# rti-team-imvia/RNb-NeuS-fork

Hardware: AMD Instinct MI355X
Metric: training rays/sec at 512 rays x 128 samples/ray (higher is better)
Workload: dtype f32; 1 GPU; DiLiGenT-MV-shaped synthetic rays, wmask_rnb.conf networks (8x256 SDF MLP + 2x256 albedo MLP), train_rnb step (render_rnb), 512 rays x (64+64) samples per GPU, 3 lights, geometric init, Adam; rays_per_gpu=512, global_rays=512, samples_per_ray=128, n_lights=3, no_albedo=False, parallelism=dp1, dp_loss=single process, deterministic=False, arithmetic=x2h, operand_bits=22, train_ops=rnb_loss_rnb + rnb_adam_step (one launch each)

## Files before the change

include/rnbneus.h:

```cpp
#ifndef RNBNEUS_H
#define RNBNEUS_H

#include <stddef.h>
#include <stdint.h>

#ifdef __cplusplus
extern "C" {
#endif

#define RNB_ABI_VERSION 5
#define RNB_MAX_LIN 16

enum {
  RNB_OK = 0,
  RNB_E_INVALID = -1,
  RNB_E_WORKSPACE = -2,
  RNB_E_HIP = -3,
  RNB_E_NULL = -4
};

typedef void* rnb_stream_t;

typedef struct rnb_model_desc {
  int32_t sdf_d_in;
  int32_t sdf_d_out;
  int32_t sdf_d_hidden;
  int32_t sdf_n_layers;
  int32_t sdf_skip_in;
  int32_t sdf_multires;
  float   sdf_scale;
  int32_t sdf_weight_norm;
  int32_t col_d_feature;
  int32_t col_d_in;
  int32_t col_d_out;
  int32_t col_d_hidden;
  int32_t col_n_layers;
  int32_t col_multires_view;
  int32_t col_squeeze_out;
  int32_t col_weight_norm;
  int32_t n_samples;
  int32_t n_importance;
  int32_t up_sample_steps;
  int32_t variant;
} rnb_model_desc;

enum {
  RNB_VARIANT_BF16 = 1,
  RNB_VARIANT_DETERMINISTIC = 2,
  RNB_VARIANT_GENERIC = 4,
  RNB_VARIANT_DW_LDS = 8,
  RNB_VARIANT_DW_STAGED = 16,
  RNB_VARIANT_X3 = 32,
  RNB_VARIANT_F32_MFMA = 64,
  RNB_VARIANT_BWD_TI_SHIFT = 8,
  RNB_VARIANT_BWD_NW_SHIFT = 10,
  RNB_VARIANT_FWD_TI_SHIFT = 12,
  RNB_VARIANT_FWD_NW_SHIFT = 14,
  RNB_VARIANT_REG_TILE = 1 << 16,
  RNB_VARIANT_LDS_TILE = 1 << 17,
  RNB_VARIANT_X2H = 1 << 18,
  RNB_VARIANT_NO_X2H = 1 << 19
};

typedef struct rnb_mlp_params {
  int32_t n_lin;
  int32_t pad_;
  const float* g[RNB_MAX_LIN];
  const float* v[RNB_MAX_LIN];
  const float* b[RNB_MAX_LIN];
} rnb_mlp_params;

typedef struct rnb_mlp_grads {
  int32_t n_lin;
  int32_t pad_;
  float* g[RNB_MAX_LIN];
  float* v[RNB_MAX_LIN];
  float* b[RNB_MAX_LIN];
} rnb_mlp_grads;

int rnb_abi_version(void);
const char* rnb_build_id(void);
const char* rnb_last_error_string(void);

int rnb_packed_floats(const rnb_model_desc* desc, int64_t* n_floats);
int rnb_weightnorm_fwd(const rnb_model_desc* desc, const rnb_mlp_params* sdf, const rnb_mlp_params* color,
                       float* packed, rnb_stream_t stream);
int rnb_weightnorm_bwd(const rnb_model_desc* desc, const rnb_mlp_params* sdf, const rnb_mlp_params* color,
                       const float* packed_grad, const rnb_mlp_grads* sdf_grads,
                       const rnb_mlp_grads* color_grads, rnb_stream_t stream);

int rnb_points_workspace_bytes(const rnb_model_desc* desc, int64_t n_points, int64_t* bytes);
int rnb_sdf_forward(const rnb_model_desc* desc, const float* packed, const float* pts, int64_t n,
                    float* sdf_out, float* feat_out, void* ws, size_t ws_bytes, rnb_stream_t stream);
int rnb_sdf_gradient(const rnb_model_desc* desc, const float* packed, const float* pts, int64_t n,
                     float* grad_out, float* sdf_out, void* ws, size_t ws_bytes, rnb_stream_t stream);
int rnb_color_forward(const rnb_model_desc* desc, const float* packed, const float* pts,
                      const float* normals, const float* feats, int64_t n, float* out, void* ws,
                      size_t ws_bytes, rnb_stream_t stream);

enum { RNB_POINTS_FEATURE = 1, RNB_POINTS_NORMAL = 2, RNB_POINTS_COLOR = 4 };
int rnb_points_grad_workspace_bytes(const rnb_model_desc* desc, int64_t n_points, int32_t flags, int64_t* bytes);
int rnb_sdf_forward_save(const rnb_model_desc* desc, const float* packed, const float* pts, int64_t n,
                         int32_t flags, float* sdf_out, float* feat_out, float* nrm_out, void* ws, size_t ws_bytes,
                         rnb_stream_t stream);
int rnb_sdf_backward(const rnb_model_desc* desc, const float* packed, int64_t n, int32_t flags, const float* sdf_bar,
                     const float* feat_bar, const float* nrm_bar, float* packed_grad, float* x_bar, void* ws,
                     size_t ws_bytes, rnb_stream_t stream);
int rnb_color_forward_save(const rnb_model_desc* desc, const float* packed, const float* pts, const float* normals,
                           const float* feats, int64_t n, float* out, void* ws, size_t ws_bytes, rnb_stream_t stream);
int rnb_color_backward(const rnb_model_desc* desc, const float* packed, int64_t n, const float* alb_bar,
                       float* packed_grad, float* feat_bar, float* nrm_bar, float* pts_bar, void* ws, size_t ws_bytes,
                       rnb_stream_t stream);

typedef struct rnb_grid_desc {
  float bound_min[3];
  float bound_max[3];
  int32_t resolution;
  int32_t x_begin, x_end;
  float out_scale;
} rnb_grid_desc;
int rnb_sdf_grid_workspace_bytes(const rnb_model_desc* desc, const rnb_grid_desc* grid, int64_t* bytes);
int rnb_sdf_grid(const rnb_model_desc* desc, const float* packed, const rnb_grid_desc* grid, float* volume,
                 void* ws, size_t ws_bytes, rnb_stream_t stream);

typedef struct rnb_sparse_grid_desc {
  int32_t brick;
  float threshold;
  float margin;
} rnb_sparse_grid_desc;
int rnb_sdf_grid_sparse_workspace_bytes(const rnb_model_desc* desc, const rnb_grid_desc* grid,
                                        const rnb_sparse_grid_desc* sparse, int64_t* bytes);
int rnb_sdf_grid_sparse_seed(const rnb_model_desc* desc, const float* packed, const rnb_grid_desc* grid,
                             const rnb_sparse_grid_desc* sparse, void* ws, size_t ws_bytes, int64_t* n_listed,
                             rnb_stream_t stream);
int rnb_sdf_grid_sparse_round(const rnb_model_desc* desc, const float* packed, const rnb_grid_desc* grid,
                              const rnb_sparse_grid_desc* sparse, float* volume, void* ws, size_t ws_bytes, int64_t first,
                              int64_t count, int64_t* n_listed, rnb_stream_t stream);
int rnb_sdf_grid_sparse_finish(const rnb_model_desc* desc, const rnb_grid_desc* grid, const rnb_sparse_grid_desc* sparse,
                               float* volume, void* ws, size_t ws_bytes, uint8_t* brick_mask, rnb_stream_t stream);

int rnb_up_sample_step(const float* rays_o, const float* rays_d, const float* z_in, const float* sdf_in,
                       int64_t B, int32_t n, int32_t n_new, float inv_s, float* new_z, int32_t* inds,
                       float* z_out, int32_t* sort_index, rnb_stream_t stream);
int rnb_gather_sdf(const float* sdf_old, const float* sdf_new, const int32_t* sort_index, int64_t B,
                   int32_t n, int32_t n_new, float* sdf_out, rnb_stream_t stream);
int rnb_sample_workspace_bytes(const rnb_model_desc* desc, int64_t B, int64_t* bytes);
int rnb_sample_rays(const rnb_model_desc* desc, const float* packed, const float* rays_o,
                    const float* rays_d, const float* near, const float* far, const float* t_rand,
                    int64_t B, float* z_vals_out, void* ws, size_t ws_bytes, rnb_stream_t stream);

enum {
  RNB_MODE_CORE = 0,
  RNB_MODE_MVPS = 1,
  RNB_FLAG_RELU_SHADING = 2,
  RNB_FLAG_NO_ALBEDO = 4,
  RNB_FLAG_LIGHT_PER_RAY = 8,
  RNB_FLAG_FORWARD_ONLY = 16,
  RNB_FLAG_INPUT_GRADS = 32
};

typedef struct rnb_render_args {
  int64_t B;
  int32_t S;
  int32_t n_lights;
  int32_t flags;
  float   cos_anneal_ratio;
  const float* rays_o;
  const float* rays_d;
  const float* z_vals;
  const float* lights_dir;
  const float* background_rgb;
  const float* variance;
  float* color_fine;
  float* weights;
  float* cdf_fine;
  float* gradients;
  float* inside_sphere;
  float* weight_sum;
  float* weight_max;
  float* s_val;
  float* gradient_error;
  float* sdf;
  float* sampled_albedo;
  float* gerr_partial;
  const float* gerr_den_global;
} rnb_render_args;

typedef struct rnb_render_grads {
  const float* color_fine;
  const float* weights;
  const float* cdf_fine;
  const float* gradients;
  const float* weight_sum;
  const float* weight_max;
  const float* s_val;
  const float* gradient_error;
} rnb_render_grads;

int rnb_render_workspace_bytes(const rnb_model_desc* desc, int64_t B, int32_t S, int32_t flags,
                               int64_t* bytes);
int rnb_render_fwd(const rnb_model_desc* desc, const float* packed, const rnb_render_args* args,
                   void* ws, size_t ws_bytes, rnb_stream_t stream);
int rnb_render_bwd(const rnb_model_desc* desc, const float* packed, const rnb_render_args* args,
                   const rnb_render_grads* gout, float* packed_grad, float* variance_grad, void* ws,
                   size_t ws_bytes, rnb_stream_t stream);

typedef struct rnb_render_input_grads {
  float* rays_o;
  float* rays_d;
  float* lights_dir;
  float* background_rgb;
  float* z_vals;
} rnb_render_input_grads;

int rnb_render_bwd_inputs(const rnb_model_desc* desc, const float* packed, const rnb_render_args* args,
                          const rnb_render_grads* gout, const rnb_render_input_grads* igrads, float* packed_grad,
                          float* variance_grad, void* ws, size_t ws_bytes, rnb_stream_t stream);

typedef struct rnb_render_maps_out {
  float* color;
  float* normal;
  float* albedo;
  float* depth;
  float* weight_sum;
  float* weight_max;
} rnb_render_maps_out;
int rnb_render_maps(const rnb_model_desc* desc, const float* packed, const rnb_render_args* args,
                    const rnb_render_maps_out* maps, void* ws, size_t ws_bytes, rnb_stream_t stream);

int rnb_algorithmic_flops(const rnb_model_desc* desc, int64_t B, int32_t flags, double* train_flops,
                          double* forward_flops);

int rnb_algorithmic_bytes(const rnb_model_desc* desc, int64_t B, int32_t flags, double* train_bytes);

int rnb_marching_cubes_workspace_bytes(int32_t nx, int32_t ny, int32_t nz, int64_t* bytes);
int rnb_marching_cubes_count(const float* volume, int32_t nx, int32_t ny, int32_t nz, float threshold,
                             void* workspace, size_t workspace_bytes, int64_t* counts, rnb_stream_t stream);
int rnb_marching_cubes_emit(const float* volume, int32_t nx, int32_t ny, int32_t nz, float threshold,
                            void* workspace, size_t workspace_bytes, int64_t n_vertices, int64_t n_triangles,
                            double* vertices, int32_t* triangles, rnb_stream_t stream);

enum { RNB_MESH_ALBEDO = 1, RNB_MESH_SWAP_RB = 2 };
typedef struct rnb_mesh_vertex_args {
  const double* grid_vertices;
  const float* points;
  int64_t V;
  float bound_min[3], bound_max[3];
  int32_t resolution;
  float level;
  int32_t refine;
  float max_step;
  int32_t flags;
  float* points_out;
  float* sdf_out;
  float* gradient_out;
  float* normal_out;
  float* albedo_out;
  uint8_t* rgb_out;
} rnb_mesh_vertex_args;
int rnb_mesh_vertex_workspace_bytes(const rnb_model_desc* desc, int64_t chunk, int32_t flags, int64_t* bytes);
int rnb_mesh_vertex_attrs(const rnb_model_desc* desc, const float* packed, const rnb_mesh_vertex_args* args,
                          int64_t chunk, void* ws, size_t ws_bytes, rnb_stream_t stream);

int rnb_gen_rays_at_view(const float* intrinsics_inv, const float* pose, const float* images,
                         const float* images_warmup, const float* mask, int32_t mask_channels,
                         const float* light_directions, const int64_t* pixels_x, const int64_t* pixels_y, int64_t B,
                         int32_t n_lights, int32_t H, int32_t W, float* data, float* true_rgb,
                         float* true_rgb_warmup, float* lights_dir, float* near, float* far, rnb_stream_t stream);

int rnb_gen_rays_grid(const float* intrinsics_inv, const float* pose, const float* tx, const float* ty, int32_t Wl,
                      int32_t Hl, int64_t first, int64_t n, const float* images, const float* images_warmup,
                      const float* mask, int32_t mask_channels, const float* light_directions, int32_t n_lights,
                      int32_t light, int32_t H, int32_t W, float* data, float* true_rgb, float* true_rgb_warmup,
                      float* lights_dir, float* near, float* far, rnb_stream_t stream);

enum { RNB_SOURCE_U8 = 0, RNB_SOURCE_U16 = 1, RNB_SOURCE_F32 = 2 };
typedef struct rnb_source_maps {
  const void* normals;
  const void* albedo;
  const void* mask;
  int32_t normals_type;
  int32_t mask_type;
  int32_t H, W, mask_channels;
  int32_t n_lights;
  float local_lights[8][3];
  float warmup_lights_cam[8][3];
} rnb_source_maps_t;
int rnb_gen_rays_at_view_from_maps(const float* intrinsics_inv, const float* pose, const rnb_source_maps_t* source,
                                   const int64_t* pixels_x, const int64_t* pixels_y, int64_t B, float* data,
                                   float* true_rgb, float* true_rgb_warmup, float* lights_dir, float* near, float* far,
                                   rnb_stream_t stream);
int rnb_gen_rays_grid_from_maps(const float* intrinsics_inv, const float* pose, const float* view_pose, const float* tx,
                                const float* ty, int32_t Wl, int32_t Hl, int64_t first, int64_t n,
                                const rnb_source_maps_t* source, int32_t light, float* data, float* true_rgb,
                                float* true_rgb_warmup, float* lights_dir, float* near, float* far, rnb_stream_t stream);

int rnb_gen_rays_camera_bwd(const float* intrinsics_inv, const float* pose, const int64_t* pixels_x,
                            const int64_t* pixels_y, int64_t B, const float* lights_dir, int32_t n_lights,
                            const float* rays_o_bar, const float* rays_d_bar, const float* lights_bar,
                            const float* near_bar, const float* far_bar, float* pose_bar, float* intrinsics_inv_bar,
                            rnb_stream_t stream);

int rnb_loss_rnb(const float* color_fine, const float* true_rgb, const float* mask, const float* weight_sum,
                 const float* gradient_error, int32_t n_lights, int64_t B, int32_t color_depth, float igr_weight,
                 float mask_weight, float* loss, float* parts, float* d_color_fine, float* d_weight_sum,
                 float* d_gradient_error, rnb_stream_t stream);
int rnb_loss_rnb_shard(const float* color_fine, const float* true_rgb, const float* mask, const float* weight_sum,
                       const float* gradient_error, int32_t n_lights, int64_t B, int32_t color_depth, float igr_weight,
                       float mask_weight, const float* batch_global, float eik_share,
                       float* loss, float* parts, float* d_color_fine, float* d_weight_sum, float* d_gradient_error,
                       rnb_stream_t stream);

int rnb_adam_step(float* param, const float* grad, float* exp_avg, float* exp_avg_sq, int64_t n, double lr,
                  double beta1, double beta2, double eps, double weight_decay, int64_t step, rnb_stream_t stream);

int rnb_render_range(const rnb_model_desc* desc, const float* packed, const void* ws, size_t ws_bytes, int64_t B, int32_t S,
                     int32_t flags, float* out, rnb_stream_t stream);

int rnb_profile_enable(int on);
int rnb_profile_collect(double* gemm_ms, int64_t* gemm_launches, double* gemm_flops);
int64_t rnb_profile_report(char* out, int64_t capacity);

#ifdef __cplusplus
}
#endif
#endif
```

rnb-neus-fork_amd/csrc/backward.hip:

```cpp
#include "gemm.hip.h"
#include "pe.hip.h"
#include "rnb_internal.h"

namespace rnb {

__global__ __launch_bounds__(64) void nbar_geb_kernel(const float* __restrict__ x4, const float* __restrict__ nrm,
                                                      const float* __restrict__ nbar_in,
                                                      const float* __restrict__ cinb, int Cinp, int blk_off,
                                                      int pen_off, int multires_view, int with_color, int multires,
                                                      int Ep, int64_t M, int64_t Mp, float* __restrict__ geb,
                                                      unsigned* __restrict__ amax) {
  extern __shared__ float tile[];
  const int lane = threadIdx.x;
  const int64_t r0 = (int64_t)blockIdx.x * 64, row = r0 + lane;
  float nb[3] = {0.f, 0.f, 0.f};
  if (with_color) {
    const int Wc = Cinp - blk_off;
    tile_load64(cinb, Cinp, r0, blk_off, Wc, tile, lane);
    __builtin_amdgcn_wave_barrier();
    if (row < M) {
      const float* g = tile + lane * (Wc + 1) + (pen_off - blk_off);
#pragma unroll
      for (int d = 0; d < 3; ++d) nb[d] = nbar_in[row * 4 + d] + g[d];
      pe_adjoint(nrm + row * 4, g, multires_view, 0, 1, nb);
    }
    __builtin_amdgcn_wave_barrier();
  } else if (row < M) {
#pragma unroll
    for (int d = 0; d < 3; ++d) nb[d] = nbar_in[row * 4 + d];
  }
  float* o = tile + lane * (Ep + 1);
  o[0] = nb[0]; o[1] = nb[1]; o[2] = nb[2];
  float gm = fmaxf(fmaxf(fabsf(nb[0]), fabsf(nb[1])), fabsf(nb[2]));
  pe_tangent(x4 + row * 4, nb, multires, 0, 1, [&](int c, float v0, float v1) {
    o[c] = v0;
    o[c + 3] = v1;
    gm = fmaxf(gm, fmaxf(fabsf(v0), fabsf(v1)));
  });
  for (int c = 3 + 6 * multires; c < Ep; ++c) o[c] = 0.f;
  if (amax != nullptr) amax_commit(amax, gm, lane);
  __builtin_amdgcn_wave_barrier();
  tile_store64(geb, Ep, r0, 0, Ep, tile, lane);
}

__global__ __launch_bounds__(512) void sdf_head_bwd_kernel(const float* __restrict__ a, const float* __restrict__ ulast,
                                                           const float* __restrict__ ucol, int ntiles,
                                                           int Hp, int H, const float* __restrict__ sbar,
                                                           float inv_scale, int64_t M, int rows_per_blk,
                                                           float* __restrict__ dwsdf, float* __restrict__ dbsdf,
                                                           float* __restrict__ part_w, float* __restrict__ part_b) {
  __shared__ double red[64][33];
  __shared__ double redb[64];
  const int tid = threadIdx.x, cg = tid & 7, ph = tid >> 3;
  const int kl = cg * 4, k0 = blockIdx.y * 32 + kl;
  const int64_t r0 = (int64_t)blockIdx.x * rows_per_blk;
  const int64_t r1 = min(M, r0 + rows_per_blk);
  double s[4] = {0.0, 0.0, 0.0, 0.0}, sb = 0.0;
#pragma unroll 4
  for (int64_t row = r0 + ph; row < r1; row += 64) {
    const float t = sbar[row] * inv_scale;
    if (cg == 0) sb += (double)t;
    const vf4 av = *reinterpret_cast<const vf4*>(a + row * Hp + k0);
    if (ulast != nullptr) {
      const vf4 uv = *reinterpret_cast<const vf4*>(ulast + row * Hp + k0);
#pragma unroll
      for (int j = 0; j < 4; ++j) s[j] += (double)(t * av[j] + uv[j]);
    } else {
#pragma unroll
      for (int j = 0; j < 4; ++j) s[j] += (double)(t * av[j]);
    }
  }
  if (ulast == nullptr && blockIdx.x == 0) {
    for (int tile = ph; tile < ntiles; tile += 64) {
      const vf4 uv = *reinterpret_cast<const vf4*>(ucol + (size_t)tile * Hp + k0);
#pragma unroll
      for (int j = 0; j < 4; ++j) s[j] += (double)uv[j];
    }
  }
#pragma unroll
  for (int j = 0; j < 4; ++j) red[ph][kl + j] = s[j];
  if (cg == 0) redb[ph] = sb;
  __syncthreads();
  if (tid < 32) {
    double t = 0.0;
    for (int q = 0; q < 64; ++q) t += red[q][tid];
    const int col = blockIdx.y * 32 + tid;
    if (part_w != nullptr) part_w[(size_t)blockIdx.x * Hp + col] = col < H ? (float)t : 0.f;
    else if (col < H) atomicAdd(dwsdf + col, (float)t);
  } else if (tid == 32 && blockIdx.y == 0) {
    double t = 0.0;
    for (int q = 0; q < 64; ++q) t += redb[q];
    if (part_b != nullptr) part_b[blockIdx.x] = (float)t;
    else atomicAdd(dbsdf, (float)t);
  }
}

__global__ void sdf_xbar_kernel(const float* __restrict__ x4, const float* __restrict__ ebar, const float* __restrict__ ge,
                                const float* __restrict__ nbar, int Ep, int multires, float scale, int64_t M,
                                float* __restrict__ xbar) {
  const int64_t row = (int64_t)blockIdx.x * blockDim.x + threadIdx.x;
  if (row >= M) return;
  const float* eb = ebar + row * Ep;
  float acc[3] = {eb[0], eb[1], eb[2]};
  const float* g = ge != nullptr ? ge + row * Ep : nullptr;
  pe_adjoint_hess(x4 + row * 4, eb, g != nullptr, g, nbar + row * 4, multires, 0, 1, acc);
#pragma unroll
  for (int d = 0; d < 3; ++d) xbar[row * 3 + d] = scale * acc[d];
}

__global__ void color_input_bwd_kernel(const float* __restrict__ cinb, int Cinp, int F, int pev, int multires_view,
                                       const float* __restrict__ p4, const float* __restrict__ n4, int64_t M,
                                       float* __restrict__ pbar, float* __restrict__ nbar) {
  const int64_t row = (int64_t)blockIdx.x * blockDim.x + threadIdx.x;
  if (row >= M) return;
  for (int which = 0; which < 2; ++which) {
    float* out = which ? nbar : pbar;
    if (out == nullptr) continue;
    const float* g = cinb + row * Cinp + F + which * pev;
    const float* v = (which ? n4 : p4) + row * 4;
    float t[3] = {g[0], g[1], g[2]};
    pe_adjoint(v, g, multires_view, 0, 1, t);
#pragma unroll
    for (int d = 0; d < 3; ++d) out[row * 3 + d] = t[d];
  }
}


static int launch_nbar_geb(const Layout& L, PointBufs& pb, bool with_color, hipStream_t s) {
  const int wt = (with_color && L.Cinp - L.F > L.Ep) ? L.Cinp - L.F : L.Ep;
  hipLaunchKernelGGL(nbar_geb_kernel, dim3(blocks_for(pb.Mp, 64)), dim3(64), (size_t)64 * (wt + 1) * sizeof(float), s,
                     pb.x, pb.nrm, pb.nbar, pb.cinb, L.Cinp, L.F, L.F + L.pev, L.multires_view, with_color ? 1 : 0,
                     L.multires, L.Ep, pb.M, pb.Mp, pb.geb, (unsigned*)nullptr);
  RNB_CHECK_LAUNCH();
  return RNB_OK;
}

static int launch_sdf_head_bwd(const Layout& L, PointBufs& pb, bool u_rows, int u_tiles, float* packed_grad, int* slabs_out,
                               hipStream_t s) {
  const int64_t M = pb.M;
  const int chunks = L.Hp / 32;
  int64_t slabs = (L.variant & RNB_VARIANT_DETERMINISTIC) ? 1 : (256 + chunks - 1) / chunks;
  const bool slab_out = dw_one_wg_runs(L, M);
  if (slab_out) slabs = kSdfHeadSlabs;
  int rows_per_blk = (int)((M + slabs - 1) / slabs);
  rows_per_blk = (rows_per_blk + 63) / 64 * 64;
  const unsigned nslab = blocks_for(M, rows_per_blk);
  hipLaunchKernelGGL(sdf_head_bwd_kernel, dim3(nslab, chunks), dim3(512), 0, s, pb.a[L.nh - 1],
                     u_rows ? (const float*)pb.u[L.nh] : (const float*)nullptr, (const float*)pb.u[L.nh], u_tiles, L.Hp,
                     L.H, pb.sbar, 1.f / L.sdf_scale, M, rows_per_blk, packed_grad + L.wsdf_off, packed_grad + L.bsdf_off,
                     slab_out ? pb.sdfh_part : nullptr, slab_out ? pb.sdfh_part + (size_t)nslab * L.Hp : nullptr);
  RNB_CHECK_LAUNCH();
  *slabs_out = slab_out ? (int)nslab : 0;
  return RNB_OK;
}

static int check_route_buffers(const Layout& L, const PointBufs& pb, const BwdParts& parts) {
  const Route& r = L.route;
  const char* missing = nullptr;
  if (r.h2 && pb.amax == nullptr) missing = "amax";
  else if (r.h2 && pb.smax == nullptr) missing = "smax";
  else if (parts.albedo && r.color == COLOR_BF16 && pb.cin8 == nullptr) missing = "cin8";
  else if (parts.albedo && r.color == COLOR_H2 && pb.col_part == nullptr) missing = "col_part";
  else if (parts.sdf && r.sdf != SDF_BF16 && dw_one_wg_runs(L, pb.M) && pb.sdfh_part == nullptr) missing = "sdfh_part";
  if (missing != nullptr) RNB_FAIL(RNB_E_WORKSPACE, "backward: this workspace has no PointBufs::%s, which the model's kernel route needs", missing);
  return RNB_OK;
}


int sweep_backward(const Layout& L, const float* packed, PointBufs& pb, bool with_color, float* packed_grad, hipStream_t s) {
  return sweep_backward_parts(L, packed, pb, BwdParts::render(with_color, false), packed_grad, s);
}

int sweep_backward_parts(const Layout& L, const float* packed, PointBufs& pb, const BwdParts& parts, float* packed_grad,
                         hipStream_t s) {
  const Route& r = L.route;
  RNB_TRY(check_route_buffers(L, pb, parts));
  RNB_TRY(dw_zero_partials(L, pb, s));
  BwdParts dw_parts = parts;
  dw_parts.albedo = parts.albedo && r.color != COLOR_BF16;
  if (parts.albedo) switch (r.color) {
    case COLOR_BF16: RNB_TRY(bf16_color_backward(L, packed, pb, packed_grad, s)); break;
    case COLOR_H2: RNB_TRY(color_h2_backward(L, packed, pb, s, parts.sdf, parts.color_inputs)); break;
    case COLOR_LAYERS: RNB_TRY(layers_color_backward(L, packed, pb, packed_grad, s)); break;
    case COLOR_NONE: RNB_FAIL(RNB_E_INVALID, "backward: the model has no albedo network");
  }
  if (!parts.sdf) return dw_backward(L, pb, dw_parts, 0, packed_grad, s);
  if (parts.normal && !(parts.albedo && r.color == COLOR_H2)) RNB_TRY(launch_nbar_geb(L, pb, parts.albedo, s));
  const bool bf = r.sdf == SDF_BF16;
  if (bf) {
    dw_parts.sdf = false;
    RNB_TRY(dw_backward(L, pb, dw_parts, 0, packed_grad, s));
  }
  int u_tiles = 0;
  if (bf) {
    RNB_TRY(bf16_ra(L, packed, pb, s));
  } else if (!parts.normal) {
    for (int l = 0; l < L.nh; ++l) RNB_CHECK_HIP(hipMemsetAsync(pb.zR[l], 0, (size_t)pb.Mp * L.Hp * sizeof(float), s));
  } else if (r.sdf == SDF_FUSED) {
    RNB_TRY(fused_ra(L, packed, pb, s, &u_tiles));
  } else {
    RNB_TRY(layers_ra(L, packed, pb, s));
  }
  int sdfh_slabs = 0;
  if (bf) RNB_TRY(bf16_sdf_head_bwd(L, pb, packed_grad, s));
  else RNB_TRY(launch_sdf_head_bwd(L, pb, parts.normal && r.sdf == SDF_LAYERS, u_tiles, packed_grad, &sdfh_slabs, s));
  switch (r.sdf) {
    case SDF_BF16: RNB_TRY(bf16_fb(L, packed, pb, parts.albedo, s)); break;
    case SDF_FUSED: RNB_TRY(fused_fb(L, packed, pb, parts.feat, s)); break;
    case SDF_LAYERS: RNB_TRY(layers_fb(L, packed, pb, parts.feat, s)); break;
  }
  if (bf) return bf16_dw_backward(L, pb, parts.albedo, packed_grad, s);
  return dw_backward(L, pb, dw_parts, sdfh_slabs, packed_grad, s);
}


int launch_sdf_xbar(const Layout& L, const float* packed, PointBufs& pb, bool with_normal, float* xbar, hipStream_t s) {
  float* ebar = nullptr;
  RNB_TRY(launch_sdf_ebar(L, packed, pb, &ebar, s));
  hipLaunchKernelGGL(sdf_xbar_kernel, dim3(blocks_for(pb.M, 256)), dim3(256), 0, s, pb.x, ebar,
                     with_normal ? (const float*)pb.ge : nullptr, pb.nbar, L.Ep, L.multires, L.sdf_scale, pb.M, xbar);
  RNB_CHECK_LAUNCH();
  return RNB_OK;
}

int launch_color_input_bwd(const Layout& L, const PointBufs& pb, float* pts_bar, float* nrm_bar, hipStream_t s) {
  if (pts_bar == nullptr && nrm_bar == nullptr) return RNB_OK;
  hipLaunchKernelGGL(color_input_bwd_kernel, dim3(blocks_for(pb.M, 256)), dim3(256), 0, s, pb.cinb, L.Cinp, L.F, L.pev,
                     L.multires_view, pb.x, pb.nrm, pb.M, pts_bar, nrm_bar);
  RNB_CHECK_LAUNCH();
  return RNB_OK;
}

}
```

rnb-neus-fork_amd/csrc/fused_bwd.hip:

```cpp
#include "fused_common.hip.h"
#include "pe.hip.h"

namespace rnb {


struct FusedBwdArgs {
  const float* packed;
  const x3raw* w3;
  SdfNetArgs net;
  float* D[RNB_MAX_LIN];
  float* gz[RNB_MAX_LIN];
  float* u[RNB_MAX_LIN + 1];
  long long M;
  float* ucol;
  float* zR[RNB_MAX_LIN];
  float* zb[RNB_MAX_LIN];
  const float* x4;
  float* nrm;
  const float* geb;
  const float* sbar;
  const float* fbar;
  int ld_fbar;
  unsigned* amax;
  const H2Tab* h2tab;
  unsigned* smax;
  float* ge_out;
};

template <int TI, int TJ = 2, bool X3 = false, class Hook = NoHook, int NP = 3>
__device__ inline void layer_mma(const float* __restrict__ X, const FusedBwdArgs& g, long long off, int K, int n0, int lane,
                                 v16f (&acc)[TI][TJ], X3Mma<TI, TJ, NP>& mm, long long off_next, Hook hook = Hook(),
                                 int hook_late = 0) {
  if constexpr (X3 && TI == 2 && TJ == 2) {
    mm.request(g.w3 + NP * off, K, n0, lane);
    mm.run(X, g.w3 + NP * off, K, n0, lane, acc, nullptr, 0, 0, hook);
  } else if constexpr (X3) mm.run(X, g.w3 + NP * off, K, n0, lane, acc, off_next >= 0 ? g.w3 + NP * off_next : nullptr, FH, n0, hook);
  else if constexpr (TI == 2 && TJ == 2) layer_mma_nt_ring<TI>(X, g.packed + off, K, n0, lane, acc, hook);
  else layer_mma_nt<TI, Hook, TJ>(X, g.packed + off, K, n0, lane, acc, hook, hook_late);
}

template <int TI, int NW = 4, bool X3 = false, bool H2 = false>
__global__ __launch_bounds__(64 * NW, (NW == 8 && TI == 2) ? 1 : 2) void fused_reverse_kernel(FusedBwdArgs g) {
  static_assert(!H2 || X3, "x2h is a form of the split-operand path");
  constexpr float SG = H2 ? kH2ActScale : 1.f;
  constexpr int WP = H2 ? 2 : 3;
  constexpr int BT = 32 * TI;
  constexpr int NT = 64 * NW;
  constexpr int TJ = 8 / NW;
  [[maybe_unused]] constexpr bool BOTH_IN_LOOP = !(TI == 2 && TJ == 2);
  constexpr int NBUF = TI == 1 ? 2 : 1;
  __shared__ __attribute__((aligned(16))) float lds[NBUF * BT * FP + BT * FEP];
  __shared__ float wmx[8];
  __shared__ int ovf[2];
  float* X = lds;
  float* Y = lds + (NBUF - 1) * BT * FP;
  float* GE = lds + NBUF * BT * FP;
  const int tid = threadIdx.x, lane = tid & 63;
  const int wave = wave_id();
  const int64_t row0 = (int64_t)blockIdx.x * BT;
  const int n0 = wave * 32 * TJ;
  [[maybe_unused]] float sg = SG, isg = 1.f / SG;
  [[maybe_unused]] float iwsv = 0.f;
  if constexpr (H2) iwsv = h2_iws_load(g.h2tab, lane);

  [[maybe_unused]] float sm = 0.f;
  {
    const float* Dl = g.D[g.net.nh - 1] + (size_t)row0 * FH;
    float* gzl = g.gz[g.net.nh - 1] + (size_t)row0 * FH;
    const float* ws = g.packed + g.net.wsdf_off;
    float m = 0.f;
    for (int idx = tid; idx < BT * FH / 4; idx += NT) {
      const int r = idx >> 6, c4 = idx & 63;
      const vf4 d = *reinterpret_cast<const vf4*>(Dl + r * FH + c4 * 4);
      const vf4 w = *reinterpret_cast<const vf4*>(ws + c4 * 4);
      const vf4 v = d * w;
      *reinterpret_cast<vf4*>(X + r * FP + c4 * 4) = v * SG;
      *reinterpret_cast<vf4*>(gzl + r * FH + c4 * 4) = v;
      if constexpr (H2) m = fmaxf(fmaxf(m, fmaxf(fabsf(v.x), fabsf(v.y))), fmaxf(fabsf(v.z), fabsf(v.w)));
    }
    for (int idx = tid; idx < BT * FEP; idx += NT) GE[idx] = 0.f;
    if constexpr (H2) {
      const bool any = __builtin_amdgcn_ballot_w64(m >= kH2ActLimit) != 0;
      if (lane == 0) wmx[wave] = any ? 1.f : 0.f;
      if (tid < 2) ovf[tid] = 0;
    }
    if constexpr (H2) sm = m;
  }
  __syncthreads();
  if constexpr (H2) {
    if (tile_max<NW>(wmx) != 0.f) {
      __syncthreads();
      sm = wave_max(sm);
      if (lane == 0) wmx[wave] = sm;
      __syncthreads();
      const float tm = tile_max<NW>(wmx);
      if (g.smax != nullptr && tid == 0) amax_tile_commit(g.smax + SMAX_GZ + g.net.nh - 1, tm);
      x2h_dyn_scale(__builtin_bit_cast(unsigned, tm), sg, isg);
      const float f = sg * (1.f / SG);
      for (int idx = tid; idx < BT * FH / 4; idx += NT) {
        vf4* q = reinterpret_cast<vf4*>(X + (idx >> 6) * FP + (idx & 63) * 4);
        *q = *q * f;
      }
      __syncthreads();
    }
  }

  v16f acc[TI][TJ];
  AuxTile<TI, TJ> aD;
  [[maybe_unused]] X3Mma<TI, TJ, WP> mm;
  if constexpr (X3 && !(TI == 2 && TJ == 2)) {
    if (g.net.nh > 1 || n0 < 64) mm.request(g.w3 + WP * g.net.wT_off[g.net.nh - 1], FH, n0, lane);
  }
  for (int l = g.net.nh - 1; l >= 1; --l) {
    [[maybe_unused]] const float INV = H2 ? isg * h2_iws_at(iwsv, l) : 1.f;
    const long long nxt = (l > 1 || n0 < 64) ? g.net.wT_off[l - 1] : -1;
    constexpr bool LATE = X3 && TI == 2 && TJ == 2;
    layer_mma<TI, TJ, X3>(X, g, g.net.wT_off[l], FH, n0, lane, acc, mm, nxt,
                     [&]() { if constexpr (!LATE) prefetch_tile<TI, TJ>(g.D[l - 1], row0, n0, lane, aD); });
    const int lane_e = opaque_lane(lane);
    const int h = lane_e >> 5;
    if constexpr (LATE) prefetch_tile<TI, TJ>(g.D[l - 1], row0, n0, lane_e, aD);
    if constexpr (NBUF == 1) lds_barrier();
    const bool is_skip = (l == g.net.skip);
    const int ksplit = is_skip ? FH - g.net.pe : FH;
    const BufRsrc rg = tile_rsrc(g.gz[l - 1] + (size_t)row0 * FH, BT * FH * 4);
    [[maybe_unused]] float gm[2] = {0.f, 0.f};
    for_each_acc_split<TI, TJ>(
        n0, lane_e, ksplit,
        [&](int tj, int ti, int r, int col, int rowc, int row) {
          const float gzv = acc[ti][tj][r] * INV * aD.v[ti][tj][r];
          Y[row * FP + col] = gzv * SG;
          bstore(rg, (unsigned)(4 * h * FH + col) * 4u, rowc * FH * 4, gzv);
          if constexpr (H2) gm[r & 1] = fmaxf(gm[r & 1], fabsf(gzv));
        },
        [&](int tj, int ti, int r, int col, int rowc, int row) {
          const float v = acc[ti][tj][r] * INV;
          float gzv;
          if (col < ksplit) {
            gzv = v * aD.v[ti][tj][r];
          } else {
            if (col < ksplit + g.net.pe) GE[row * FEP + (col - ksplit)] = v;
            gzv = 0.f;
          }
          Y[row * FP + col] = gzv * SG;
          bstore(rg, (unsigned)(4 * h * FH + col) * 4u, rowc * FH * 4, gzv);
          if constexpr (H2) gm[r & 1] = fmaxf(gm[r & 1], fabsf(gzv));
        });
    if constexpr (H2) h2_raise_flag(fmaxf(gm[0], gm[1]), &ovf[l & 1], lane_e);
    lds_barrier();
    if constexpr (H2) {
      sg = SG;
      isg = 1.f / SG;
      if (h2_flag_up(&ovf[l & 1])) {
        const float m = wave_max(fmaxf(gm[0], gm[1]));
        if (lane_e == 0) wmx[wave] = m;
        lds_barrier();
        const float tm = tile_max<NW>(wmx);
        if (g.smax != nullptr && tid == 0) amax_tile_commit(g.smax + SMAX_GZ + l - 1, tm);
        if (tid == 0) ovf[l & 1] = 0;
        x2h_dyn_scale(__builtin_bit_cast(unsigned, tm), sg, isg);
        const float f = sg * (1.f / SG);
        for_each_acc<TI, TJ>(n0, lane_e, [&](int tj, int ti, int r, int col, int rowc, int row) { Y[row * FP + col] *= f; });
        lds_barrier();
      }
    }
    if constexpr (NBUF == 2) { float* t = X; X = Y; Y = t; }
  }
  if (n0 < 64) {
    [[maybe_unused]] const float INV = H2 ? isg * h2_iws_at(iwsv, 0) : 1.f;
    layer_mma<TI, TJ, X3>(X, g, g.net.wT_off[0], FH, n0, lane, acc, mm, -1);
    for_each_acc<TI, TJ>(n0, lane, [&](int tj, int ti, int r, int col, int rowc, int row) {
      if (col < g.net.pe) GE[row * FEP + col] += acc[ti][tj][r] * INV;
    });
  }
  __syncthreads();
  if (tid < BT) {
    const int64_t row = row0 + tid;
    const float* ge = GE + tid * FEP;
    float n[3] = {ge[0], ge[1], ge[2]};
    pe_adjoint(g.x4 + row * 4, ge, g.net.multires, 0, 1, n);
    g.nrm[row * 4] = n[0]; g.nrm[row * 4 + 1] = n[1]; g.nrm[row * 4 + 2] = n[2]; g.nrm[row * 4 + 3] = 0.f;
    if (g.ge_out != nullptr)
      for (int c = 0; c < g.net.pe; ++c) g.ge_out[row * g.net.Ep + c] = ge[c];
  }
}

template <int TI, int NW = 4, bool X3 = false>
__global__ __launch_bounds__(64 * NW, (NW == 8 && TI == 2) ? 1 : 2) void fused_ra_kernel(FusedBwdArgs g) {
  constexpr int BT = 32 * TI;
  constexpr int NT = 64 * NW;
  constexpr int TJ = 8 / NW;
  [[maybe_unused]] constexpr bool BOTH_IN_LOOP = !(TI == 2 && TJ == 2);
  constexpr int NBUF = TI == 1 ? 2 : 1;
  __shared__ __attribute__((aligned(16))) float lds[NBUF * BT * FP + BT * FEP];
  float* X = lds;
  float* Y = lds + (NBUF - 1) * BT * FP;
  float* E = lds + NBUF * BT * FP;
  __shared__ float wmx[2][8];
  const int tid = threadIdx.x, lane = tid & 63;
  const int wave = wave_id();
  const int64_t row0 = (int64_t)blockIdx.x * BT;
  const int n0 = wave * 32 * TJ;

  float gm = 0.f;
  for (int idx = tid; idx < BT * g.net.Ep; idx += NT) {
    const int r = idx / g.net.Ep, c = idx - r * g.net.Ep;
    const float v = g.geb[(row0 + r) * g.net.Ep + c];
    X[r * FP + c] = v;
    if (c < FEP) E[r * FEP + c] = v;
    gm = fmaxf(gm, fabsf(v));
  }
  if (g.amax != nullptr) {
#pragma unroll
    for (int o = 32; o > 0; o >>= 1) gm = fmaxf(gm, __shfl_xor(gm, o, 64));
    if (lane == 0) wmx[1][wave] = gm;
  }
  __syncthreads();
  if (g.amax != nullptr && tid == 0) {
    float m = wmx[1][0];
    for (int w = 1; w < NW; ++w) m = fmaxf(m, wmx[1][w]);
    amax_tile_commit(g.amax + AMAX_U, m);
  }

  v16f acc[TI][TJ];
  AuxTile<TI, TJ> aD, aG;
  [[maybe_unused]] X3Mma<TI, TJ> mm;
  if constexpr (X3 && !(TI == 2 && TJ == 2)) mm.request(g.w3 + 3 * g.net.w_off[0], g.net.Kp[0], n0, lane);
  for (int l = 0; l < g.net.nh; ++l) {
    layer_mma<TI, TJ, X3>(X, g, g.net.w_off[l], g.net.Kp[l], n0, lane, acc, mm, l + 1 < g.net.nh ? g.net.w_off[l + 1] : -1,
                     [&]() {
                       if constexpr (!(X3 && !BOTH_IN_LOOP)) prefetch_tile<TI, TJ>(g.D[l], row0, n0, lane, aD);
                       if constexpr (BOTH_IN_LOOP) prefetch_tile<TI, TJ>(g.gz[l], row0, n0, lane, aG);
                     });
    const int lane_e = opaque_lane(lane);
    const int h = lane_e >> 5;
    if constexpr (X3 && !BOTH_IN_LOOP) prefetch_tile<TI, TJ>(g.D[l], row0, n0, lane_e, aD);
    if constexpr (!BOTH_IN_LOOP) prefetch_tile<TI, TJ>(g.gz[l], row0, n0, lane_e, aG);
    if constexpr (NBUF == 1) lds_barrier();
    const int n_real = g.net.n_real[l];
    const bool pe_tail = (l + 1 == g.net.skip);
    const BufRsrc rzR = tile_rsrc(g.zR[l] + (size_t)row0 * FH, BT * FH * 4);
    if (l + 1 == g.net.nh && g.ucol != nullptr) {
      float cs[TJ];
#pragma unroll
      for (int tj = 0; tj < TJ; ++tj) cs[tj] = 0.f;
      for_each_acc<TI, TJ>(n0, lane_e, [&](int tj, int ti, int r, int col, int rowc, int row) {
        const float v = acc[ti][tj][r];
        const float un = col < n_real ? v * aD.v[ti][tj][r] : 0.f;
        const float zr = col < n_real ? ((v - un) * aG.v[ti][tj][r]) * 100.f : 0.f;
        bstore(rzR, (unsigned)(4 * h * FH + col) * 4u, rowc * FH * 4, zr);
        cs[tj] += (row0 + row < g.M) ? un : 0.f;
      });
#pragma unroll
      for (int tj = 0; tj < TJ; ++tj) {
        const float tot = cs[tj] + __shfl_xor(cs[tj], 32, 64);
        if (lane_e < 32) g.ucol[(size_t)blockIdx.x * FH + n0 + tj * 32 + lane_e] = tot;
      }
      break;
    }
    const BufRsrc ru = tile_rsrc(g.u[l + 1] + (size_t)row0 * FH, BT * FH * 4);
    float um[2] = {0.f, 0.f};
    for_each_acc_split<TI, TJ>(
        n0, lane_e, n_real,
        [&](int tj, int ti, int r, int col, int rowc, int row) {
          const unsigned voff = (unsigned)(4 * h * FH + col) * 4u;
          const unsigned soff = rowc * FH * 4;
          const float v = acc[ti][tj][r];
          const float un = v * aD.v[ti][tj][r];
          const float zr = ((v - un) * aG.v[ti][tj][r]) * 100.f;
          Y[row * FP + col] = un;
          bstore(rzR, voff, soff, zr);
          bstore(ru, voff, soff, un);
          um[r & 1] = fmaxf(um[r & 1], fabsf(un));
        },
        [&](int tj, int ti, int r, int col, int rowc, int row) {
          const unsigned voff = (unsigned)(4 * h * FH + col) * 4u;
          const unsigned soff = rowc * FH * 4;
          const float v = acc[ti][tj][r];
          float zr, un;
          if (col < n_real) {
            un = v * aD.v[ti][tj][r];
            zr = ((v - un) * aG.v[ti][tj][r]) * 100.f;
          } else {
            zr = 0.f;
            un = (pe_tail && col < n_real + g.net.pe) ? E[row * FEP + (col - n_real)] : 0.f;
          }
          Y[row * FP + col] = un;
          bstore(rzR, voff, soff, zr);
          bstore(ru, voff, soff, un);
          um[r & 1] = fmaxf(um[r & 1], fabsf(un));
        });
    if (g.amax != nullptr) {
      float m = fmaxf(um[0], um[1]);
#pragma unroll
      for (int o = 32; o > 0; o >>= 1) m = fmaxf(m, __shfl_xor(m, o, 64));
      if (lane_e == 0) wmx[l & 1][wave] = m;
    }
    lds_barrier();
    if (g.amax != nullptr && tid == 0) {
      float m = wmx[l & 1][0];
      for (int w = 1; w < NW; ++w) m = fmaxf(m, wmx[l & 1][w]);
      amax_tile_commit(g.amax + AMAX_U + l + 1, m);
    }
    if constexpr (NBUF == 2) { float* t = X; X = Y; Y = t; }
  }
}

template <int TI, int NW = 4, bool X3 = false>
__global__ __launch_bounds__(64 * NW, (NW == 8 && TI == 2) ? 1 : 2) void fused_fb_kernel(FusedBwdArgs g) {
  constexpr int BT = 32 * TI;
  constexpr int NT = 64 * NW;
  constexpr int TJ = 8 / NW;
  [[maybe_unused]] constexpr bool BOTH_IN_LOOP = !(TI == 2 && TJ == 2);
  constexpr int NBUF = TI == 1 ? 2 : 1;
  __shared__ __attribute__((aligned(16))) float lds[NBUF * BT * FP];
  float* X = lds;
  float* Y = lds + (NBUF - 1) * BT * FP;
  const int tid = threadIdx.x, lane = tid & 63;
  const int wave = wave_id();
  const int64_t row0 = (int64_t)blockIdx.x * BT;
  const int n0 = wave * 32 * TJ;

  v16f acc[TI][TJ];
  AuxTile<TI, TJ> aD, aZ;
  [[maybe_unused]] X3Mma<TI, TJ> mm;
  if constexpr (X3 && !(TI == 2 && TJ == 2)) {
    if (g.fbar != nullptr) mm.request(g.w3 + 3 * g.net.wfT_off, FH, n0, lane);
    else if (g.net.nh > 1) mm.request(g.w3 + 3 * g.net.wT_off[g.net.nh - 1], FH, n0, lane);
  }
  constexpr bool LATE = X3 && TI == 2 && TJ == 2;
  if constexpr (!LATE) {
    prefetch_tile<TI, TJ>(g.D[g.net.nh - 1], row0, n0, lane, aD);
    prefetch_tile<TI, TJ>(g.zR[g.net.nh - 1], row0, n0, lane, aZ);
  }
  for (int ti_ = 0; ti_ < TI; ++ti_) for (int tj_ = 0; tj_ < TJ; ++tj_) for (int r_ = 0; r_ < 16; ++r_) acc[ti_][tj_][r_] = 0.f;
  if (g.fbar != nullptr) {
    const float* fb = g.fbar + (size_t)row0 * g.ld_fbar;
    for (int idx = tid; idx < BT * FH / 4; idx += NT) {
      const int r = idx >> 6, c4 = idx & 63;
      *reinterpret_cast<vf4*>(X + r * FP + c4 * 4) = *reinterpret_cast<const vf4*>(fb + (size_t)r * g.ld_fbar + c4 * 4);
    }
    __syncthreads();
    layer_mma<TI, TJ, X3>(X, g, g.net.wfT_off, FH, n0, lane, acc, mm, g.net.nh > 1 ? g.net.wT_off[g.net.nh - 1] : -1);
    if constexpr (NBUF == 1) lds_barrier();
  }
  if constexpr (LATE) {
    prefetch_tile<TI, TJ>(g.D[g.net.nh - 1], row0, n0, lane, aD);
    prefetch_tile<TI, TJ>(g.zR[g.net.nh - 1], row0, n0, lane, aZ);
  }
  for (int l = g.net.nh - 1; l >= 0; --l) {
    const int lane_e = opaque_lane(lane);
    const int h = lane_e >> 5;
    const int n_real = g.net.n_real[l];
    const bool head = (l == g.net.nh - 1);
    const BufRsrc rzb = tile_rsrc(g.zb[l] + (size_t)row0 * FH, BT * FH * 4);
    if (head) {
      for_each_acc<TI, TJ>(n0, lane_e, [&](int tj, int ti, int r, int col, int rowc, int row) {
        acc[ti][tj][r] = fmaf(g.sbar[row0 + row] * g.net.inv_scale, g.packed[g.net.wsdf_off + col], acc[ti][tj][r]);
      });
    }
    for_each_acc_split<TI, TJ>(
        n0, lane_e, n_real,
        [&](int tj, int ti, int r, int col, int rowc, int row) {
          const float zb = fmaf(acc[ti][tj][r], aD.v[ti][tj][r], aZ.v[ti][tj][r]);
          Y[row * FP + col] = zb;
          bstore(rzb, (unsigned)(4 * h * FH + col) * 4u, rowc * FH * 4, zb);
          acc[ti][tj][r] = zb;
        },
        [&](int tj, int ti, int r, int col, int rowc, int row) {
          const float zb = col < n_real ? fmaf(acc[ti][tj][r], aD.v[ti][tj][r], aZ.v[ti][tj][r]) : 0.f;
          Y[row * FP + col] = zb;
          bstore(rzb, (unsigned)(4 * h * FH + col) * 4u, rowc * FH * 4, zb);
          acc[ti][tj][r] = zb;
        });
    if (g.amax != nullptr) {
      const long long left = g.M - row0;
      amax_commit(g.amax + AMAX_ZB + l, acc_absmax<TI, TJ>(acc, lane_e, left >= BT ? BT : (int)(left < 0 ? 0 : left)), lane_e);
    }
    if (l == 0) break;
    lds_barrier();
    if constexpr (NBUF == 2) { float* t = X; X = Y; Y = t; }
    layer_mma<TI, TJ, X3>(X, g, g.net.wT_off[l], FH, n0, lane, acc, mm, l > 1 ? g.net.wT_off[l - 1] : -1,
                     [&]() {
                       if constexpr (!(X3 && !BOTH_IN_LOOP)) prefetch_tile<TI, TJ>(g.D[l - 1], row0, n0, lane, aD);
                       if constexpr (BOTH_IN_LOOP) prefetch_tile<TI, TJ>(g.zR[l - 1], row0, n0, lane, aZ);
                     });
    if constexpr (X3 && !BOTH_IN_LOOP) prefetch_tile<TI, TJ>(g.D[l - 1], row0, n0, opaque_lane(lane), aD);
    if constexpr (!BOTH_IN_LOOP) prefetch_tile<TI, TJ>(g.zR[l - 1], row0, n0, opaque_lane(lane), aZ);
    if constexpr (NBUF == 1) lds_barrier();
  }
}

template <int NW>
__global__ __launch_bounds__(64 * NW, NW == 8 ? 1 : 2) void fused_fb_h2_kernel(FusedBwdArgs g) {
  constexpr int TI = 2, BT = 64, NT = 64 * NW, TJ = 8 / NW;
  __shared__ __attribute__((aligned(16))) float lds[BT * FP];
  __shared__ float wm[2][8];
  float* X = lds;
  const int tid = threadIdx.x, lane = tid & 63;
  const int wave = wave_id();
  const int64_t row0 = (int64_t)blockIdx.x * BT;
  const int n0 = wave * 32 * TJ;
  const long long left = g.M - row0;
  const int rows_ok = left >= BT ? BT : (int)(left < 0 ? 0 : left);

  v16f acc[TI][TJ];
  AuxTile<TI, TJ> aD, aZ;
  X3Mma<TI, TJ, 2> mm;
  constexpr bool LATE = TJ == 2;
  if constexpr (!LATE) {
    if (g.fbar != nullptr) mm.request(g.w3 + 2 * g.net.wfT_off, FH, n0, lane);
    else if (g.net.nh > 1) mm.request(g.w3 + 2 * g.net.wT_off[g.net.nh - 1], FH, n0, lane);
    prefetch_tile<TI, TJ>(g.D[g.net.nh - 1], row0, n0, lane, aD);
    prefetch_tile<TI, TJ>(g.zR[g.net.nh - 1], row0, n0, lane, aZ);
  }
  for (int ti_ = 0; ti_ < TI; ++ti_) for (int tj_ = 0; tj_ < TJ; ++tj_) for (int r_ = 0; r_ < 16; ++r_) acc[ti_][tj_][r_] = 0.f;
  float unscale = 1.f;
  const float iwsv = h2_iws_load(g.h2tab, lane);
  if (g.fbar != nullptr) {
    const float* fb = g.fbar + (size_t)row0 * g.ld_fbar;
    float m = 0.f;
    for (int idx = tid; idx < BT * FH / 4; idx += NT) {
      const int r = idx >> 6, c4 = idx & 63;
      const vf4 v = *reinterpret_cast<const vf4*>(fb + (size_t)r * g.ld_fbar + c4 * 4);
      *reinterpret_cast<vf4*>(X + r * FP + c4 * 4) = v;
      if (r < rows_ok) m = fmaxf(fmaxf(m, fmaxf(fabsf(v.x), fabsf(v.y))), fmaxf(fabsf(v.z), fabsf(v.w)));
    }
    m = wave_max(m);
    if (lane == 0) wm[1][wave] = m;
    __syncthreads();
    float s, inv;
    tile_scale<NW>(wm[1], s, inv);
    for (int idx = tid; idx < BT * FH / 4; idx += NT) {
      const int r = idx >> 6, c4 = idx & 63;
      vf4* q = reinterpret_cast<vf4*>(X + r * FP + c4 * 4);
      *q = *q * s;
    }
    __syncthreads();
    if constexpr (LATE) mm.request(g.w3 + 2 * g.net.wfT_off, FH, n0, lane);
    mm.run(X, g.w3 + 2 * g.net.wfT_off, FH, n0, lane, acc, (!LATE && g.net.nh > 1) ? g.w3 + 2 * g.net.wT_off[g.net.nh - 1] : nullptr, FH, n0);
    unscale = inv * h2_iws_at(iwsv, g.net.nh);
  }
  if constexpr (LATE) {
    prefetch_tile<TI, TJ>(g.D[g.net.nh - 1], row0, n0, lane, aD);
    prefetch_tile<TI, TJ>(g.zR[g.net.nh - 1], row0, n0, lane, aZ);
  }
  for (int l = g.net.nh - 1; l >= 0; --l) {
    const int lane_e = opaque_lane(lane);
    const int h = lane_e >> 5;
    const int n_real = g.net.n_real[l];
    const bool head = (l == g.net.nh - 1);
    const int par = l & 1;
    const BufRsrc rzb = tile_rsrc(g.zb[l] + (size_t)row0 * FH, BT * FH * 4);
    if (head) {
      for_each_acc<TI, TJ>(n0, lane_e, [&](int tj, int ti, int r, int col, int rowc, int row) {
        acc[ti][tj][r] = fmaf(g.sbar[row0 + row] * g.net.inv_scale, g.packed[g.net.wsdf_off + col], acc[ti][tj][r] * unscale);
      });
      unscale = 1.f;
    }
    for_each_acc_split<TI, TJ>(
        n0, lane_e, n_real,
        [&](int tj, int ti, int r, int col, int rowc, int row) {
          const float zb = fmaf(acc[ti][tj][r] * unscale, aD.v[ti][tj][r], aZ.v[ti][tj][r]);
          bstore(rzb, (unsigned)(4 * h * FH + col) * 4u, rowc * FH * 4, zb);
          acc[ti][tj][r] = zb;
        },
        [&](int tj, int ti, int r, int col, int rowc, int row) {
          const float zb = col < n_real ? fmaf(acc[ti][tj][r] * unscale, aD.v[ti][tj][r], aZ.v[ti][tj][r]) : 0.f;
          bstore(rzb, (unsigned)(4 * h * FH + col) * 4u, rowc * FH * 4, zb);
          acc[ti][tj][r] = zb;
        });
    {
      const float mr = wave_max(acc_absmax<TI, TJ>(acc, lane_e, rows_ok));
      if (lane_e == 0) wm[par][wave] = mr;
    }
    lds_barrier();
    float s, inv;
    const float tmax = tile_scale<NW>(wm[par], s, inv);
    if (tid == 0 && g.amax != nullptr) amax_tile_commit(g.amax + AMAX_ZB + l, tmax);
    if (l == 0) break;
    for_each_acc<TI, TJ>(n0, lane_e, [&](int tj, int ti, int r, int col, int rowc, int row) {
      X[row * FP + col] = acc[ti][tj][r] * s;
    });
    lds_barrier();
    if constexpr (LATE) {
      mm.request(g.w3 + 2 * g.net.wT_off[l], FH, n0, lane);
      mm.run(X, g.w3 + 2 * g.net.wT_off[l], FH, n0, lane, acc, nullptr, 0, 0);
      prefetch_tile<TI, TJ>(g.D[l - 1], row0, n0, opaque_lane(lane), aD);
      prefetch_tile<TI, TJ>(g.zR[l - 1], row0, n0, opaque_lane(lane), aZ);
    } else {
      mm.run(X, g.w3 + 2 * g.net.wT_off[l], FH, n0, lane, acc, l > 1 ? g.w3 + 2 * g.net.wT_off[l - 1] : nullptr, FH, n0, [&]() {
        prefetch_tile<TI, TJ>(g.D[l - 1], row0, n0, lane, aD);
        prefetch_tile<TI, TJ>(g.zR[l - 1], row0, n0, lane, aZ);
      });
    }
    unscale = inv * h2_iws_at(iwsv, l);
  }
}

static void fill_args(const Layout& L, const float* packed, PointBufs& pb, FusedBwdArgs& g) {
  memset(&g, 0, sizeof(g));
  g.net = sdf_net_args(L);
  g.packed = packed;
  g.w3 = reinterpret_cast<const x3raw*>(packed + L.total);
  for (int l = 0; l < L.nh; ++l) {
    g.D[l] = pb.D[l];
    g.gz[l] = pb.gz[l];
    g.zR[l] = pb.zR[l];
    g.zb[l] = pb.zb[l];
  }
  for (int l = 1; l <= L.nh; ++l) g.u[l] = pb.u[l];
  g.M = pb.M;
  g.x4 = pb.x;
  g.nrm = pb.nrm;
  g.geb = pb.geb;
  g.sbar = pb.sbar;
  g.amax = is_x2h(L) ? pb.amax : nullptr;
  g.h2tab = is_x2h(L) ? h2_tab(L, packed) : nullptr;
}

template <class F>
static void pick_tile(const Layout& L, const PointBufs& pb, F&& f) {
  const int kt = L.knob(RNB_VARIANT_BWD_TI_SHIFT), kw = L.knob(RNB_VARIANT_BWD_NW_SHIFT);
  const int ti = kt == 1 || kt == 2 ? kt : (is_x3(L) ? 2 : 1), nw = kw == 1 ? 4 : kw == 2 ? 8 : (is_x3(L) ? 4 : 8);
  pick_c<2, 1>(ti, [&](auto ti_c) {
    pick_c<8, 4>(nw, [&](auto nw_c) { f(ti_c, nw_c, dim3((unsigned)(pb.Mp / (32 * ti_c))), dim3(64 * nw_c)); });
  });
}

int fused_reverse(const Layout& L, const float* packed, PointBufs& pb, hipStream_t s, bool store_ge) {
  FusedBwdArgs g;
  fill_args(L, packed, pb, g);
  g.ge_out = store_ge ? pb.ge : nullptr;
  if (is_x2h(L)) {
    g.w3 = x2h_mirror(L, packed);
    g.smax = pb.smax;
  }
  ProfScope prof(sdf_sweep_flops(L, pb.M, 0, false, false), s, "R_sweep");
  pick_tile(L, pb, [&](auto ti_c, auto nw_c, dim3 grid, dim3 block) {
    pick_c<2, 1, 0>(is_x2h(L) ? 2 : is_x3(L) ? 1 : 0, [&](auto ar_c) {
      constexpr int AR = decltype(ar_c)::value;
      hipLaunchKernelGGL((fused_reverse_kernel<decltype(ti_c)::value, decltype(nw_c)::value, AR >= 1, AR == 2>), grid, block, 0, s, g);
    });
  });
  RNB_CHECK_LAUNCH();
  return RNB_OK;
}

int fused_ra(const Layout& L, const float* packed, PointBufs& pb, hipStream_t s, int* u_tiles) {
  FusedBwdArgs g;
  fill_args(L, packed, pb, g);
  ProfScope prof(sdf_sweep_flops(L, pb.M, 0, false, false), s, "RA_sweep");
  pick_tile(L, pb, [&](auto ti_c, auto nw_c, dim3 grid, dim3 block) {
    if (u_tiles != nullptr) {
      g.ucol = pb.u[L.nh];
      *u_tiles = (int)grid.x;
    }
    pick_c<1, 0>(is_x3(L), [&](auto x3_c) {
      hipLaunchKernelGGL((fused_ra_kernel<decltype(ti_c)::value, decltype(nw_c)::value, decltype(x3_c)::value != 0>), grid, block, 0, s, g);
    });
  });
  RNB_CHECK_LAUNCH();
  return RNB_OK;
}

int fused_fb(const Layout& L, const float* packed, PointBufs& pb, bool with_color, hipStream_t s) {
  FusedBwdArgs g;
  fill_args(L, packed, pb, g);
  g.fbar = with_color ? pb.cinb : nullptr;
  g.ld_fbar = L.Cinp;
  ProfScope prof(sdf_sweep_flops(L, pb.M, 1, false, with_color), s, "FB_sweep");
  pick_tile(L, pb, [&](auto ti_c, auto nw_c, dim3 grid, dim3 block) {
    constexpr int TI = decltype(ti_c)::value, NW = decltype(nw_c)::value;
    if constexpr (TI == 2) {
      if (is_x2h(L)) {
        g.w3 = x2h_mirror(L, packed);
        hipLaunchKernelGGL((fused_fb_h2_kernel<NW>), grid, block, 0, s, g);
        return;
      }
    }
    pick_c<1, 0>(is_x3(L), [&](auto x3_c) {
      hipLaunchKernelGGL((fused_fb_kernel<TI, NW, decltype(x3_c)::value != 0>), grid, block, 0, s, g);
    });
  });
  RNB_CHECK_LAUNCH();
  return RNB_OK;
}

}
```

rnb-neus-fork_amd/csrc/layout.hip:

```cpp
#include <stdarg.h>

#include "rnb_internal.h"

namespace rnb {

static thread_local char g_err[512] = "";

void set_error(const char* fmt, ...) {
  va_list ap;
  va_start(ap, fmt);
  vsnprintf(g_err, sizeof(g_err), fmt, ap);
  va_end(ap);
}
const char* last_error() { return g_err; }

static void place(Lin& l, int N, int K, float scale, int64_t& off) {
  l.N = N;
  l.K = K;
  l.Np = pad32(N);
  l.Kp = pad32(K);
  l.scale = scale;
  l.w_off = off;
  off += (int64_t)l.Np * l.Kp;
  l.b_off = off;
  off += l.Np;
  l.wT_off = -1;
}
static void place_transpose(Lin& l, int64_t& off) {
  l.wT_off = off;
  off += (int64_t)l.Kp * l.Np;
}

int make_layout(const rnb_model_desc* d, Layout* L) {
  if (!d || !L) RNB_FAIL(RNB_E_NULL, "null desc");
  memset(L, 0, sizeof(*L));
  if (d->sdf_d_in != 3) RNB_FAIL(RNB_E_INVALID, "sdf_d_in must be 3 (got %d)", d->sdf_d_in);
  if (d->sdf_n_layers < 1 || d->sdf_n_layers + 1 > RNB_MAX_LIN)
    RNB_FAIL(RNB_E_INVALID, "sdf_n_layers out of range (%d)", d->sdf_n_layers);
  if (d->sdf_d_hidden < 1 || d->sdf_d_out < 1) RNB_FAIL(RNB_E_INVALID, "bad sdf widths");
  if (d->sdf_multires < 0 || d->sdf_multires > 16) RNB_FAIL(RNB_E_INVALID, "bad sdf_multires");
  if (!(d->sdf_scale > 0.f)) RNB_FAIL(RNB_E_INVALID, "sdf_scale must be positive");
  L->variant = d->variant;
  if (d->variant & ~0xFFF7F) RNB_FAIL(RNB_E_INVALID, "unknown bits in rnb_model_desc.variant (0x%x)", d->variant);
  L->nh = d->sdf_n_layers;
  L->multires = d->sdf_multires;
  L->pe = 3 * (1 + 2 * d->sdf_multires);
  L->Ep = pad32(L->pe);
  L->H = d->sdf_d_hidden;
  L->Hp = pad32(L->H);
  L->skip = d->sdf_skip_in;
  L->sdf_scale = d->sdf_scale;
  if (L->skip >= 0 && (L->skip < 1 || L->skip > L->nh - 1))
    RNB_FAIL(RNB_E_INVALID, "sdf_skip_in must be in [1, n_layers-1] or -1 (got %d)", L->skip);
  if (L->skip >= 0 && L->H - L->pe < 1) RNB_FAIL(RNB_E_INVALID, "d_hidden too small for the skip connection");
  int64_t off = 0;
  for (int l = 0; l < L->nh; ++l) {
    const int K = l == 0 ? L->pe : L->H;
    const int N = (l + 1 == L->skip) ? L->H - L->pe : L->H;
    L->hid[l].N = N;
    L->hid[l].K = K;
    L->hid[l].Np = L->Hp;
    L->hid[l].Kp = pad32(K);
    L->hid[l].scale = l == L->skip ? 0.70710678118654752440f : 1.f;
    L->hid[l].w_off = off;
    off += (int64_t)L->Hp * L->hid[l].Kp;
    L->hid[l].b_off = off;
    off += L->Hp;
    place_transpose(L->hid[l], off);
  }
  L->F = d->sdf_d_out - 1;
  L->Fp = pad32(L->F > 0 ? L->F : 1);
  place(L->feat, L->F > 0 ? L->F : 0, L->H, 1.f, off);
  if (L->F <= 0) { L->feat.Np = 0; }
  else place_transpose(L->feat, off);
  L->wsdf_off = off;
  off += L->Hp;
  L->bsdf_off = off;
  off += kPad;
  L->nc = d->col_n_layers;
  L->multires_view = d->col_multires_view;
  if (L->F > 0) {
    if (d->col_n_layers < 1 || d->col_n_layers + 1 > RNB_MAX_LIN) RNB_FAIL(RNB_E_INVALID, "bad col_n_layers");
    if (d->col_d_feature != L->F) RNB_FAIL(RNB_E_INVALID, "col_d_feature (%d) != sdf_d_out-1 (%d)", d->col_d_feature, L->F);
    if (d->col_d_in != 6) RNB_FAIL(RNB_E_INVALID, "col_d_in must be 6 in no_view_dir mode");
    if (d->col_d_out < 1 || d->col_d_out > 4) RNB_FAIL(RNB_E_INVALID, "col_d_out must be 1..4");
    L->pev = 3 * (1 + 2 * d->col_multires_view);
    L->Cin = L->F + 2 * L->pev;
    L->Cinp = pad32(L->Cin);
    L->Hc = d->col_d_hidden;
    L->Hcp = pad32(L->Hc);
    L->Co = d->col_d_out;
    L->Cop = kPad;
    L->squeeze = d->col_squeeze_out;
    for (int l = 0; l < L->nc; ++l) {
      place(L->col[l], L->Hc, l == 0 ? L->Cin : L->Hc, 1.f, off);
      place_transpose(L->col[l], off);
    }
    place(L->colo, L->Co, L->Hc, 1.f, off);
  }
  L->total = (off + 31) / 32 * 32;
  L->total_all = L->total;
  if (d->variant & RNB_VARIANT_BF16) {
    if (!fused_supported(*L))
      RNB_FAIL(RNB_E_INVALID, "RNB_VARIANT_BF16 needs the 256-wide SDF network shape (d_hidden 256, feature width 225..256)");
    if (L->Ep != 64) RNB_FAIL(RNB_E_INVALID, "RNB_VARIANT_BF16 needs 33..40 positional-encoding columns (multires 5 or 6), got %d", L->pe);
    if (L->skip == 1) RNB_FAIL(RNB_E_INVALID, "RNB_VARIANT_BF16 does not support a skip connection at layer 1");
    if (d->variant & RNB_VARIANT_GENERIC) RNB_FAIL(RNB_E_INVALID, "RNB_VARIANT_BF16 and RNB_VARIANT_GENERIC exclude each other");
    L->total_all = L->total + L->total / 2;
  }
  if (d->variant & RNB_VARIANT_X3) {
    if (d->variant & (RNB_VARIANT_BF16 | RNB_VARIANT_GENERIC | RNB_VARIANT_F32_MFMA))
      RNB_FAIL(RNB_E_INVALID, "RNB_VARIANT_X3 excludes RNB_VARIANT_BF16, RNB_VARIANT_GENERIC and RNB_VARIANT_F32_MFMA");
    if (!fused_supported(*L)) RNB_FAIL(RNB_E_INVALID, "RNB_VARIANT_X3 needs the 256-wide SDF network shape");
  }
  if (!(d->variant & (RNB_VARIANT_BF16 | RNB_VARIANT_GENERIC | RNB_VARIANT_F32_MFMA)) && fused_supported(*L))
    L->variant |= RNB_VARIANT_X3;
  if (L->variant & RNB_VARIANT_X3)
    L->total_all = L->total + L->total / 2 * 3;
  if ((d->variant & RNB_VARIANT_REG_TILE) && (d->variant & RNB_VARIANT_LDS_TILE))
    RNB_FAIL(RNB_E_INVALID, "RNB_VARIANT_REG_TILE and RNB_VARIANT_LDS_TILE exclude each other");
  if ((d->variant & RNB_VARIANT_X2H) && (d->variant & RNB_VARIANT_NO_X2H))
    RNB_FAIL(RNB_E_INVALID, "RNB_VARIANT_X2H and RNB_VARIANT_NO_X2H exclude each other");
  if ((d->variant & RNB_VARIANT_X2H) && !(L->variant & RNB_VARIANT_X3))
    RNB_FAIL(RNB_E_INVALID, "RNB_VARIANT_X2H is a form of the x3 path (256-wide SDF network, fp32)");
  if ((L->variant & RNB_VARIANT_X3) && !(d->variant & RNB_VARIANT_NO_X2H)) L->variant |= RNB_VARIANT_X2H;
  L->h2tab_off = -1;
  if (L->variant & RNB_VARIANT_X2H) {
    L->total_all += L->total;
    L->h2tab_off = L->total_all;
    L->total_all += 256;
    if (L->nh + 1 + L->nc > kH2TabSlots) RNB_FAIL(RNB_E_INVALID, "too many layers for the x2h scale table");
  }
  Route& r = L->route;
  r.sdf = is_bf16(*L) ? SDF_BF16 : (!(L->variant & RNB_VARIANT_GENERIC) && fused_supported(*L)) ? SDF_FUSED : SDF_LAYERS;
  r.color = (is_bf16(*L) && bf16_color_supported(*L)) ? COLOR_BF16
            : (r.sdf == SDF_FUSED && color_h2_supported(*L)) ? COLOR_H2
            : L->F > 0 ? COLOR_LAYERS : COLOR_NONE;
  r.h2 = is_x2h(*L) && r.sdf == SDF_FUSED;
  return RNB_OK;
}

void carve_points(const Layout& L, Carver& c, int64_t M, int mode, PointBufs* pb) {
  memset(pb, 0, sizeof(*pb));
  pb->M = M;
  pb->Mp = pad_rows(M);
  const int64_t Mp = pb->Mp;
  const bool bf = L.route.sdf == SDF_BF16;
  auto take_state = [&](int64_t n) { return bf ? reinterpret_cast<float*>(c.take<uint16_t>(n)) : c.take<float>(n); };
  pb->x = c.take<float>(Mp * 4);
  pb->e = c.take<float>(Mp * L.Ep);
  for (int l = 0; l < L.nh; ++l) pb->a[l] = take_state(Mp * L.Hp);
  pb->sdf = c.take<float>(Mp);
  pb->smax = c.take<unsigned>(SMAX_SLOTS);
  if (mode & (PM_WITH_NORMAL | PM_WITH_COLOR | PM_WITH_BACKWARD)) {
    if (!(mode & PM_NO_REVERSE))
      for (int l = 0; l < L.nh; ++l) pb->gz[l] = take_state(Mp * L.Hp);
    for (int l = 0; l < L.nh; ++l) pb->D[l] = take_state(Mp * L.Hp);
    pb->ge = c.take<float>(Mp * L.Ep);
    pb->nrm = c.take<float>(Mp * 4);
  }
  if (mode & PM_WITH_COLOR) {
    pb->cin = c.take<float>(Mp * L.Cinp);
    for (int l = 0; l < L.nc; ++l) pb->ac[l] = c.take<float>(Mp * L.Hcp);
    pb->alb = c.take<float>(Mp * 4);
    if (L.route.color == COLOR_H2) pb->ac0_mask = c.take<unsigned>(Mp / 64 * 256 * 2);
    if (L.route.color == COLOR_BF16) {
      pb->cin8 = c.take<uint16_t>(Mp * L.Cinp);
      for (int l = 0; l < L.nc; ++l) pb->ac8[l] = c.take<uint16_t>(Mp * L.Hcp);
    }
  }
  if (mode & PM_WITH_BACKWARD) {
    if (!(mode & PM_NO_REVERSE))
      for (int l = 1; l <= L.nh; ++l) pb->u[l] = take_state(Mp * L.Hp);
    for (int l = 0; l < L.nh; ++l) pb->zR[l] = take_state(Mp * L.Hp);
    for (int l = 0; l < L.nh; ++l) pb->zb[l] = take_state(Mp * L.Hp);
    if (bf) {
      pb->u0_k8 = c.take<uint16_t>(Mp * L.Ep);
      pb->fbar_k8 = c.take<uint16_t>(Mp * L.Hp);
    }
    pb->geb = c.take<float>(Mp * L.Ep);
    pb->amax = c.take<unsigned>(AMAX_SLOTS);
    pb->sbar = c.take<float>(Mp);
    pb->nbar = c.take<float>(Mp * 4);
    pb->albbar = c.take<float>(Mp * 4);
    if (mode & PM_WITH_COLOR) {
      for (int l = 0; l < L.nc; ++l) pb->zc[l] = c.take<float>(Mp * L.Hcp);
      pb->cinb = c.take<float>(Mp * L.Cinp);
      if (L.route.color == COLOR_BF16)
        for (int l = 0; l < L.nc; ++l) pb->zc8[l] = c.take<uint16_t>(Mp * L.Hcp);
    }
    {
      const bool wc = (mode & PM_WITH_COLOR) != 0;
      pb->dw_part_floats = dw_workspace_floats(L, M, wc, &pb->dw_slab_off);
      pb->dw_part = c.take<float>(pb->dw_part_floats > 0 ? pb->dw_part_floats : 64);
      if (wc && L.route.color == COLOR_H2) pb->col_part = c.take<float>(color_h2_part_floats(L, M));
      pb->sdfh_part = c.take<float>((int64_t)kSdfHeadSlabs * (L.Hp + 1));
    }
  }
}

}
```

rnb-neus-fork_amd/csrc/prof.hip:

```cpp
#include <stdio.h>
#include <string.h>

#include <vector>

#include "rnb_internal.h"

namespace rnb {

struct ProfState {
  bool on = false;
  std::vector<hipEvent_t> pool;
  size_t used = 0;
  std::vector<double> flops;
  std::vector<const char*> tag;
};
static ProfState g_prof;

bool prof_enabled() { return g_prof.on; }

void prof_begin(double flops, hipStream_t s, const char* tag) {
  ProfState& p = g_prof;
  if (p.used + 2 > p.pool.size()) {
    for (int i = 0; i < 2; ++i) {
      hipEvent_t e;
      if (hipEventCreate(&e) != hipSuccess) { p.on = false; return; }
      p.pool.push_back(e);
    }
  }
  p.flops.push_back(flops);
  p.tag.push_back(tag);
  (void)hipEventRecord(p.pool[p.used], s);
}
void prof_end(hipStream_t s) {
  ProfState& p = g_prof;
  (void)hipEventRecord(p.pool[p.used + 1], s);
  p.used += 2;
}

int profile_enable(int on) {
  g_prof.on = on != 0;
  g_prof.used = 0;
  g_prof.flops.clear();
  g_prof.tag.clear();
  return RNB_OK;
}

struct ProfClass { const char* tag; double ms, flops; int64_t n; };
static std::vector<ProfClass> g_classes;

int profile_collect(double* ms, int64_t* launches, double* flops) {
  ProfState& p = g_prof;
  double t = 0, f = 0;
  const size_t n = p.used / 2;
  g_classes.clear();
  for (size_t i = 0; i < n; ++i) {
    float e = 0.f;
    RNB_CHECK_HIP(hipEventElapsedTime(&e, p.pool[2 * i], p.pool[2 * i + 1]));
    t += e;
    f += p.flops[i];
    const char* tg = p.tag[i] ? p.tag[i] : "other";
    size_t c = 0;
    while (c < g_classes.size() && strcmp(g_classes[c].tag, tg) != 0) ++c;
    if (c == g_classes.size()) g_classes.push_back(ProfClass{tg, 0.0, 0.0, 0});
    g_classes[c].ms += e;
    g_classes[c].flops += p.flops[i];
    g_classes[c].n += 1;
  }
  if (ms) *ms = t;
  if (launches) *launches = (int64_t)n;
  if (flops) *flops = f;
  p.used = 0;
  p.flops.clear();
  p.tag.clear();
  return RNB_OK;
}

int64_t profile_report(char* out, int64_t cap) {
  int64_t need = 0;
  for (const ProfClass& c : g_classes) {
    char line[160];
    const int k = snprintf(line, sizeof line, "%s %.6f %lld %.6e\n", c.tag, c.ms, (long long)c.n, c.flops);
    if (out && need + k < cap) memcpy(out + need, line, (size_t)k);
    need += k;
  }
  if (out && cap > 0) out[need < cap ? need : cap - 1] = 0;
  return need + 1;
}

}
```

rnb-neus-fork_amd/csrc/rnb_internal.h:

```cpp
#pragma once
#include <hip/hip_runtime.h>
#include <stdint.h>
#include <stdio.h>
#include <string.h>

#include <type_traits>

#include "../../include/rnbneus.h"

namespace rnb {

constexpr int kPad = 32;
constexpr int kRowPad = 128;
inline int pad32(int x) { return (x + kPad - 1) / kPad * kPad; }
inline int64_t pad_rows(int64_t m) { return (m + kRowPad - 1) / kRowPad * kRowPad; }
inline unsigned blocks_for(int64_t n, int per) { return (unsigned)((n + per - 1) / per); }

void set_error(const char* fmt, ...);
#define RNB_FAIL(code, ...)        \
  do {                             \
    ::rnb::set_error(__VA_ARGS__); \
    return (code);                 \
  } while (0)
#define RNB_CHECK_HIP(expr)                                                          \
  do {                                                                               \
    hipError_t e_ = (expr);                                                          \
    if (e_ != hipSuccess) RNB_FAIL(RNB_E_HIP, "%s: %s", #expr, hipGetErrorString(e_)); \
  } while (0)
#define RNB_CHECK_LAUNCH() RNB_CHECK_HIP(hipGetLastError())
#define RNB_TRY(expr)          \
  do {                         \
    int rc_ = (expr);          \
    if (rc_ != RNB_OK) return rc_; \
  } while (0)

struct Lin {
  int N, K;
  int Np, Kp;
  int64_t w_off;
  int64_t wT_off;
  int64_t b_off;
  float scale;
};
inline double mm_flops(int64_t M, const Lin& ln) { return 2.0 * (double)M * ln.N * ln.K; }

enum SdfRoute { SDF_LAYERS, SDF_FUSED, SDF_BF16 };
enum ColorRoute { COLOR_NONE, COLOR_LAYERS, COLOR_H2, COLOR_BF16 };
struct Route {
  SdfRoute sdf;
  ColorRoute color;
  bool h2;
};

struct Layout {
  int nh;
  int pe;
  int Ep;
  int H, Hp;
  int skip;
  Lin hid[RNB_MAX_LIN];
  int F, Fp;
  Lin feat;
  int64_t wsdf_off;
  int64_t bsdf_off;
  float sdf_scale;
  int multires;
  int nc;
  int pev;
  int Cin, Cinp;
  int Hc, Hcp;
  int Co, Cop;
  Lin col[RNB_MAX_LIN];
  Lin colo;
  int multires_view;
  int squeeze;
  int64_t total;
  int64_t total_all;
  int64_t h2tab_off;
  int variant;
  int knob(int shift) const { return (variant >> shift) & 3; }
  Route route;
};

int make_layout(const rnb_model_desc* d, Layout* L);

struct SdfNetArgs {
  int nh, skip, pe, multires, Ep;
  float scale, inv_scale;
  int n_real[RNB_MAX_LIN];
  int Kp[RNB_MAX_LIN];
  long long w_off[RNB_MAX_LIN], b_off[RNB_MAX_LIN], wT_off[RNB_MAX_LIN];
  long long wsdf_off, bsdf_off;
  int F, Cinp;
  long long wf_off, bf_off, wfT_off;
};
inline SdfNetArgs sdf_net_args(const Layout& L) {
  SdfNetArgs n;
  memset(&n, 0, sizeof(n));
  n.nh = L.nh; n.skip = L.skip; n.pe = L.pe; n.multires = L.multires; n.Ep = L.Ep;
  n.scale = L.sdf_scale;
  n.inv_scale = 1.f / L.sdf_scale;
  for (int l = 0; l < L.nh; ++l) {
    n.n_real[l] = L.hid[l].N;
    n.Kp[l] = L.hid[l].Kp;
    n.w_off[l] = L.hid[l].w_off;
    n.b_off[l] = L.hid[l].b_off;
    n.wT_off[l] = L.hid[l].wT_off;
  }
  n.wsdf_off = L.wsdf_off;
  n.bsdf_off = L.bsdf_off;
  n.F = L.F;
  n.Cinp = L.Cinp;
  n.wf_off = L.feat.w_off; n.bf_off = L.feat.b_off; n.wfT_off = L.feat.wT_off;
  return n;
}
inline double sdf_sweep_flops(const Layout& L, int64_t M, int first, bool sdf_row, bool feat) {
  double fl = 0;
  for (int l = first; l < L.nh; ++l) fl += mm_flops(M, L.hid[l]);
  if (sdf_row) fl += 2.0 * (double)M * L.H;
  if (feat) fl += 2.0 * (double)M * L.F * L.H;
  return fl;
}

template <int V0, int... Vs, class F>
inline void pick_c(int v, F&& f) {
  if constexpr (sizeof...(Vs) == 0) f(std::integral_constant<int, V0>{});
  else if (v == V0) f(std::integral_constant<int, V0>{});
  else pick_c<Vs...>(v, f);
}

#if defined(__HIPCC__)
__device__ inline float max_nan(float a, float b) { return a != a ? a : (b != b ? b : fmaxf(a, b)); }
__device__ inline float min_nan(float a, float b) { return a != a ? a : (b != b ? b : fminf(a, b)); }
__device__ inline float clamp_nan(float x, float lo, float hi) { return x != x ? x : fminf(fmaxf(x, lo), hi); }
__device__ inline float relu_nan(float x) { return x < 0.f ? 0.f : x; }

__device__ inline float linspace_at(float start, float end, int steps, int i) {
  if (steps == 1) return start;
  const float step = (end - start) / (float)(steps - 1);
  return i < steps / 2 ? fmaf(step, (float)i, start) : fmaf(-step, (float)(steps - 1 - i), end);
}
#endif

enum { GRID_OFF = 0, GRID_DENSE = 1, GRID_BRICKS = 2, GRID_LATTICE = 3 };
struct GridGen {
  int on;
  int res, x_begin;
  float bmin[3], bmax[3];
  float out_scale;
  const int32_t* bricks;
  int bs, nb;
  int rows_per_brick;
  int64_t family_rows;
};
inline int64_t family_rows_of(const GridGen* g, int64_t Mp) { return g != nullptr && g->family_rows != 0 ? g->family_rows : Mp; }

#if defined(__HIPCC__)
__device__ inline int64_t grid_locate(const GridGen& g, int64_t row, int64_t M, int& ix, int& iy, int& iz) {
  if (row >= M) return -1;
  if (g.on == GRID_DENSE) {
    int64_t r = row;
    iz = (int)(r % g.res);
    r /= g.res;
    iy = (int)(r % g.res);
    ix = (int)(r / g.res) + g.x_begin;
    return row;
  }
  if (g.on == GRID_BRICKS) {
    const int n1 = g.bs + 1;
    const int l = (int)(row % g.rows_per_brick);
    if (l >= n1 * n1 * n1) return -1;
    int b = g.bricks[row / g.rows_per_brick];
    const int bz = b % g.nb;
    b /= g.nb;
    ix = (b / g.nb) * g.bs + l / (n1 * n1);
    iy = (b % g.nb) * g.bs + (l / n1) % n1;
    iz = bz * g.bs + l % n1;
    if (ix >= g.res || iy >= g.res || iz >= g.res) return -1;
    return ((int64_t)ix * g.res + iy) * g.res + iz;
  }
  const int nl = g.nb + 1;
  int64_t r = row;
  iz = min((int)(r % nl) * g.bs, g.res - 1);
  r /= nl;
  iy = min((int)(r % nl) * g.bs, g.res - 1);
  ix = min((int)(r / nl) * g.bs, g.res - 1);
  return row;
}
__device__ inline int64_t grid_out_index(const GridGen& g, int64_t row, int64_t M) {
  if (g.on == GRID_DENSE) return row < M ? row : -1;
  int ix, iy, iz;
  return grid_locate(g, row, M, ix, iy, iz);
}

__device__ inline void sweep_point(const GridGen& grid, const float* pts, int64_t row, int64_t M, float scale, float (&x)[3]) {
  x[0] = x[1] = x[2] = 0.f;
  if (row < M) {
    if (grid.on) {
      const int res = grid.res;
      int ix, iy, iz;
      if (grid_locate(grid, row, M, ix, iy, iz) >= 0) {
        x[0] = linspace_at(grid.bmin[0], grid.bmax[0], res, ix) * scale;
        x[1] = linspace_at(grid.bmin[1], grid.bmax[1], res, iy) * scale;
        x[2] = linspace_at(grid.bmin[2], grid.bmax[2], res, iz) * scale;
      }
    } else {
      x[0] = pts[row * 3] * scale;
      x[1] = pts[row * 3 + 1] * scale;
      x[2] = pts[row * 3 + 2] * scale;
    }
  }
}
__device__ inline void sweep_store_sdf(const GridGen& grid, float* sdf, int64_t row0, int r, int64_t M, float v) {
  if (!grid.on) sdf[row0 + r] = v;
  else {
    const int64_t o = grid_out_index(grid, row0 + r, M);
    if (o >= 0) sdf[o] = v * grid.out_scale;
  }
}
#endif

struct Carver {
  char* base;
  size_t cap;
  size_t off = 0;
  bool ok = true;
  Carver(void* p, size_t bytes) : base((char*)p), cap(bytes) {}
  template <class T>
  T* take(int64_t n) {
    size_t bytes = ((size_t)n * sizeof(T) + 255) / 256 * 256;
    T* p = (T*)(base ? base + off : nullptr);
    off += bytes;
    if (base && off > cap) ok = false;
    return p;
  }
};

constexpr int kH2TabSlots = 48;
struct H2Tab {
  unsigned wmax[kH2TabSlots];
  float ws[kH2TabSlots];
  float iws[kH2TabSlots];
};
static_assert(sizeof(H2Tab) <= 256 * sizeof(float), "the packed buffer reserves 256 floats for the table");
inline int h2_id_hid(int l) { return l; }

struct PointBufs {
  int64_t M, Mp;
  float* x;
  float* e;
  float* a[RNB_MAX_LIN];
  float* D[RNB_MAX_LIN];
  float* gz[RNB_MAX_LIN];
  float* ge;
  float* sdf;
  float* nrm;
  float* cin;
  float* ac[RNB_MAX_LIN];
  float* alb;
  float* u[RNB_MAX_LIN];
  float* zR[RNB_MAX_LIN];
  float* zb[RNB_MAX_LIN];
  float* geb;
  float* zc[RNB_MAX_LIN];
  float* cinb;
  float* sbar;
  float* nbar;
  float* albbar;
  void* u0_k8;
  void* cin8;
  void* ac8[RNB_MAX_LIN];
  void* zc8[RNB_MAX_LIN];
  void* fbar_k8;
  unsigned* amax;
  unsigned* smax;
  float* dw_part;
  int64_t dw_part_floats;
  int64_t dw_slab_off;
  unsigned* ac0_mask;
  float* col_part;
  float* sdfh_part;
};

enum { AMAX_ZB = 0, AMAX_U = RNB_MAX_LIN, AMAX_ZC = 2 * RNB_MAX_LIN + 1, AMAX_CINB = 3 * RNB_MAX_LIN + 1, AMAX_SLOTS = 3 * RNB_MAX_LIN + 2 };
enum { SMAX_A = 0, SMAX_GZ = RNB_MAX_LIN, SMAX_E = 2 * RNB_MAX_LIN, SMAX_CIN = 2 * RNB_MAX_LIN + 1, SMAX_AC = 2 * RNB_MAX_LIN + 2,
       SMAX_SLOTS = 3 * RNB_MAX_LIN + 2 };
inline unsigned* h2_slot(const Layout& L, unsigned* slots, int i) { return L.route.h2 && slots != nullptr ? slots + i : nullptr; }
enum PointMode { PM_SDF_ONLY = 0, PM_WITH_NORMAL = 1, PM_WITH_COLOR = 2, PM_WITH_BACKWARD = 4, PM_NO_REVERSE = 8 };
void carve_points(const Layout& L, Carver& c, int64_t M, int mode, PointBufs* pb);

int launch_pe_points(const Layout& L, const float* pts, int64_t M, PointBufs& pb, hipStream_t s);
int sweep_forward(const Layout& L, const float* packed, PointBufs& pb, bool need_feat, bool need_gz_last,
                  float* feat_dense, hipStream_t s);
int sweep_reverse(const Layout& L, const float* packed, PointBufs& pb, hipStream_t s);
int sweep_color(const Layout& L, const float* packed, PointBufs& pb, const float* pts, const float* nrm, int nrm_ld,
                hipStream_t s);
int layers_color_backward(const Layout& L, const float* packed, PointBufs& pb, float* packed_grad, hipStream_t s);
int layers_ra(const Layout& L, const float* packed, PointBufs& pb, hipStream_t s);
int layers_fb(const Layout& L, const float* packed, PointBufs& pb, bool with_feat, hipStream_t s);
int launch_sdf_ebar(const Layout& L, const float* packed, PointBufs& pb, float** ebar, hipStream_t s);

int launch_copy_cols(const float* src, int ld, int ncols, int64_t M, float* out, hipStream_t s);
int launch_fill_cols(const float* src, int ncols, int64_t M, int64_t Mp, int ld, float* dst, hipStream_t s);
int launch_grid_points(const GridGen& g, int64_t first, int64_t n, float* pts, hipStream_t s);
int launch_scale_copy(const float* src, float scale, int64_t n, float* dst, hipStream_t s);
int launch_grid_scatter(const GridGen& g, const float* src, int64_t first, int64_t n, float* dst, hipStream_t s);

struct MeshPointsSrc {
  const double* grid;
  const float* pts;
  double rm1;
  float span[3], bmin[3];
};
struct MeshOut {
  float* points;
  float* sdf;
  float* gradient;
  float* normal;
  float* albedo;
  uint8_t* rgb;
  int Co;
  int swap_rb;
};
int launch_mesh_points(const MeshPointsSrc& src, int64_t first, int64_t n, float* pts, hipStream_t s);
int launch_mesh_newton(const float* sdf, const float* nrm, int64_t n, float level, float max_step, float* pts, hipStream_t s);
int launch_mesh_attrs(const float* pts, const PointBufs& pb, int64_t first, int64_t n, const MeshOut& o, hipStream_t s);

struct SparseGeom {
  int res, bs, nb, nl;
  float thr;
  float seed_dist;
};
int launch_sparse_classify(const SparseGeom& sg, const float* lattice, uint32_t* state, int32_t* list, int64_t* n_listed,
                           hipStream_t s);
int launch_sparse_grow(const SparseGeom& sg, const float* volume, int64_t first, int64_t count, uint32_t* state, int32_t* list,
                       int64_t* n_listed, hipStream_t s);
int launch_sparse_fill(const SparseGeom& sg, const float* lattice, const uint32_t* state, float* volume, hipStream_t s);
int launch_absmax_rows(const float* x, int64_t n, unsigned* slot, hipStream_t s);
int launch_range_report(const Layout& L, const float* packed, const PointBufs& pb, bool with_color, bool with_backward, float* out,
                        hipStream_t s);

struct BwdParts {
  bool albedo;
  bool sdf;
  bool feat;
  bool normal;
  bool color_inputs;
  static BwdParts render(bool with_color, bool keep_color_inputs) { return {with_color, true, with_color, true, keep_color_inputs}; }
  static BwdParts sdf_points(bool feat, bool normal) { return {false, true, feat, normal, false}; }
  static BwdParts color_points(bool inputs) { return {true, false, false, false, inputs}; }
};
int sweep_backward(const Layout& L, const float* packed, PointBufs& pb, bool with_color, float* packed_grad, hipStream_t s);
int sweep_backward_parts(const Layout& L, const float* packed, PointBufs& pb, const BwdParts& parts, float* packed_grad,
                         hipStream_t s);
int launch_sdf_xbar(const Layout& L, const float* packed, PointBufs& pb, bool with_normal, float* xbar, hipStream_t s);
int launch_color_input_bwd(const Layout& L, const PointBufs& pb, float* pts_bar, float* nrm_bar, hipStream_t s);
int64_t dw_workspace_floats(const Layout& L, int64_t M, bool with_color, int64_t* slab_off);
bool dw_one_wg_runs(const Layout& L, int64_t M);
int dw_zero_partials(const Layout& L, const PointBufs& pb, hipStream_t s);
int dw_backward(const Layout& L, const PointBufs& pb, const BwdParts& parts, int sdfh_slabs, float* packed_grad, hipStream_t s);
int fused_reverse(const Layout& L, const float* packed, PointBufs& pb, hipStream_t s, bool store_ge = false);
int fused_ra(const Layout& L, const float* packed, PointBufs& pb, hipStream_t s, int* u_tiles = nullptr);
int fused_fb(const Layout& L, const float* packed, PointBufs& pb, bool with_color, hipStream_t s);

bool fused_supported(const Layout& L);
int fused_forward(const Layout& L, const float* packed, const float* pts, int64_t M, PointBufs& pb, bool save,
                  bool need_feat, hipStream_t s, const GridGen* grid = nullptr);
bool sweep_mv_supported(const Layout& L);
int sweep_mv_forward(const Layout& L, const float* packed, const float* pts, int64_t M, PointBufs& pb, bool save,
                     bool need_feat, hipStream_t s, const GridGen* grid = nullptr);
constexpr bool kRegTileDefault = false;
inline bool use_reg_tile(const Layout& L, int64_t Mp) {
  if (!sweep_mv_supported(L) || (L.variant & RNB_VARIANT_LDS_TILE)) return false;
  if (L.variant & RNB_VARIANT_REG_TILE) return true;
  return kRegTileDefault && Mp >= 128 * 200;
}

inline bool is_x3(const Layout& L) { return (L.variant & RNB_VARIANT_X3) != 0; }
inline bool is_x2h(const Layout& L) { return is_x3(L) && (L.variant & RNB_VARIANT_X2H) != 0; }
inline unsigned short* x2h_mirror(const Layout& L, float* packed) {
  return reinterpret_cast<unsigned short*>(packed + L.total + L.total / 2 * 3);
}
inline const unsigned short* x2h_mirror(const Layout& L, const float* packed) {
  return reinterpret_cast<const unsigned short*>(packed + L.total + L.total / 2 * 3);
}
inline const H2Tab* h2_tab(const Layout& L, const float* packed) {
  return L.h2tab_off >= 0 ? reinterpret_cast<const H2Tab*>(packed + L.h2tab_off) : nullptr;
}
inline H2Tab* h2_tab(const Layout& L, float* packed) {
  return L.h2tab_off >= 0 ? reinterpret_cast<H2Tab*>(packed + L.h2tab_off) : nullptr;
}
int x3_pack_weights(const Layout& L, float* packed, hipStream_t s);

bool color_h2_supported(const Layout& L);
int color_h2_forward(const Layout& L, const float* packed, PointBufs& pb, const float* pts, const float* nrm, hipStream_t s);
int color_h2_backward(const Layout& L, const float* packed, PointBufs& pb, hipStream_t s, bool sdf = true, bool keep_pe = false);
int64_t color_h2_part_floats(const Layout& L, int64_t M);
constexpr int kSdfHeadSlabs = 64;

inline bool is_bf16(const Layout& L) { return (L.variant & RNB_VARIANT_BF16) != 0; }
int bf16_pack_weights(const Layout& L, float* packed, hipStream_t s);
int bf16_forward(const Layout& L, const float* packed, const float* pts, int64_t M, PointBufs& pb, bool save, bool need_feat,
                 hipStream_t s, const GridGen* grid = nullptr, bool feat_k8 = false);
int bf16_reverse(const Layout& L, const float* packed, PointBufs& pb, hipStream_t s);
int bf16_ra(const Layout& L, const float* packed, PointBufs& pb, hipStream_t s);
int bf16_fb(const Layout& L, const float* packed, PointBufs& pb, bool with_color, hipStream_t s);
bool bf16_color_supported(const Layout& L);
int bf16_color_forward(const Layout& L, const float* packed, PointBufs& pb, const float* pts, hipStream_t s);
int bf16_color_backward(const Layout& L, const float* packed, PointBufs& pb, float* packed_grad, hipStream_t s);
int bf16_sdf_head_bwd(const Layout& L, PointBufs& pb, float* packed_grad, hipStream_t s);
int bf16_dw_backward(const Layout& L, PointBufs& pb, bool with_color, float* packed_grad, hipStream_t s);
int64_t bf16_dw_floats(const Layout& L, int64_t M, bool with_color);

int launch_up_sample_step(const float* rays_o, const float* rays_d, const float* z_in, const float* sdf_old,
                          const float* sdf_new, const int32_t* gather_index, int n_old_for_gather,
                          int64_t B, int n, int n_new, float inv_s, float* new_z, int32_t* inds,
                          float* z_out, int32_t* sort_index, float* new_pts, float* sdf_sorted_out,
                          hipStream_t s);

struct CompArgs {
  int64_t B;
  int S, L, C;
  int flags;
  float cos_anneal;
  const float* rays_d;
  const float* pts;
  const float* dists;
  const float* sdf;
  const float* nrm;
  const float* alb;
  const float* lights;
  const float* bg;
  const float* variance;
  float* color_fine;
  float* weights;
  float* cdf;
  float* gradients;
  float* inside;
  float* weight_sum;
  float* weight_max;
  float* s_val;
  float* gerr_part;
  float* gerr;
  float* gerr_den;
  float* gerr_partial;
  float* sdf_out;
  float* albedo_out;
};

struct CompBwdArgs {
  CompArgs f;
  const float* weights;
  const float* g_color;
  const float* g_weights;
  const float* g_cdf;
  const float* g_gradients;
  const float* g_weight_sum;
  const float* g_weight_max;
  const float* g_s_val;
  const float* g_gerr;
  const float* gerr_den;
  const float* gerr_den_global;
  float* sbar;
  float* nbar;
  float* albbar;
  float* invs_part;
  float* dvar;
  unsigned* amax_to_zero;
  float* ig_cos_d;
  float* ig_light;
  float* ig_bg;
  float* ig_dists;
};

struct CompMapsArgs {
  CompArgs f;
  const float* z;
  float* normal;
  float* albedo;
  float* depth;
};

int launch_fine_points(const float* rays_o, const float* rays_d, const float* z, int64_t B, int S, float sample_dist,
                       float* pts, float* dists, unsigned* smax_to_zero, hipStream_t s);
int launch_composite_fwd(const CompArgs& a, hipStream_t s);
int launch_composite_maps(const CompMapsArgs& g, hipStream_t s);
int launch_composite_bwd(const CompBwdArgs& g, hipStream_t s);
constexpr int kMaxS = 512;
constexpr int kMaxRenderLights = 8;
struct RayAdjArgs {
  int64_t B;
  int S;
  const float* pts;
  const float* dists;
  const float* z;
  const float* rays_d;
  const float* x4;
  const float* ebar;
  const float* ge;
  const float* nbar;
  const float* nrm;
  const float* cinb;
  int Ep, multires, Cinp, F, pev, multires_view;
  float scale;
  const float* cos_d;
  const float* dists_bar;
  float* o_bar;
  float* d_bar;
  float* z_bar;
};
int launch_ray_input_adjoint(const RayAdjArgs& r, hipStream_t s);
int launch_sum_over_rays(const float* part, int64_t B, int nvec, float* out, hipStream_t s);

constexpr int kMaxZ = 512;
constexpr int kMaxNew = 64;
int launch_z_init(const float* rays_o, const float* rays_d, const float* near, const float* far,
                  const float* t_rand, int64_t B, int n, float* z, float* pts, hipStream_t s);
int launch_gather_sdf(const float* sdf_old, const float* sdf_new, const int32_t* index, int64_t B, int n, int n_new,
                      float* out, hipStream_t s);

int weightnorm_fwd(const rnb_model_desc* d, const Layout& L, const rnb_mlp_params* sdf, const rnb_mlp_params* color,
                   float* packed, hipStream_t s);
int weightnorm_bwd(const rnb_model_desc* d, const Layout& L, const rnb_mlp_params* sdf, const rnb_mlp_params* color,
                   const float* pgrad, const rnb_mlp_grads* gs, const rnb_mlp_grads* gc, hipStream_t s);
const char* last_error();

bool prof_enabled();
void prof_begin(double flops, hipStream_t s, const char* tag);
void prof_end(hipStream_t s);
int profile_enable(int on);
int profile_collect(double* ms, int64_t* launches, double* flops);
int64_t profile_report(char* out, int64_t cap);
struct ProfScope {
  hipStream_t s;
  bool on;
  ProfScope(double flops, hipStream_t st, const char* tag = nullptr) : s(st), on(prof_enabled()) {
    if (on) prof_begin(flops, s, tag);
  }
  ~ProfScope() {
    if (on) prof_end(s);
  }
};

}
```

rnb-neus-fork_amd/native.py:

```python
from __future__ import annotations

import ctypes as C
import os

_HERE = os.path.dirname(os.path.abspath(__file__))
LIB_PATH = os.path.join(_HERE, "librnbneus_hip.so")
ABI_VERSION = 5
MAX_LIN = 16

MODE_CORE = 0
MODE_MVPS = 1
FLAG_RELU_SHADING = 2
FLAG_NO_ALBEDO = 4
FLAG_LIGHT_PER_RAY = 8
FLAG_FORWARD_ONLY = 16
FLAG_INPUT_GRADS = 32
MAX_RENDER_LIGHTS = 8

POINTS_FEATURE = 1
POINTS_NORMAL = 2
POINTS_COLOR = 4

MESH_ALBEDO = 1
MESH_SWAP_RB = 2

VARIANT_BF16 = 1
VARIANT_DETERMINISTIC = 2
VARIANT_GENERIC = 4
VARIANT_DW_LDS = 8
VARIANT_DW_STAGED = 16
VARIANT_X3 = 32
VARIANT_F32_MFMA = 64
VARIANT_BWD_TI_SHIFT, VARIANT_BWD_NW_SHIFT, VARIANT_FWD_TI_SHIFT, VARIANT_FWD_NW_SHIFT = 8, 10, 12, 14
VARIANT_REG_TILE = 1 << 16
VARIANT_LDS_TILE = 1 << 17
VARIANT_X2H = 1 << 18
VARIANT_NO_X2H = 1 << 19

c_float_p = C.c_void_p


class ModelDesc(C.Structure):
    _fields_ = [
        ("sdf_d_in", C.c_int32), ("sdf_d_out", C.c_int32), ("sdf_d_hidden", C.c_int32),
        ("sdf_n_layers", C.c_int32), ("sdf_skip_in", C.c_int32), ("sdf_multires", C.c_int32),
        ("sdf_scale", C.c_float), ("sdf_weight_norm", C.c_int32),
        ("col_d_feature", C.c_int32), ("col_d_in", C.c_int32), ("col_d_out", C.c_int32),
        ("col_d_hidden", C.c_int32), ("col_n_layers", C.c_int32), ("col_multires_view", C.c_int32),
        ("col_squeeze_out", C.c_int32), ("col_weight_norm", C.c_int32),
        ("n_samples", C.c_int32), ("n_importance", C.c_int32), ("up_sample_steps", C.c_int32),
        ("variant", C.c_int32),
    ]


class MlpParams(C.Structure):
    _fields_ = [("n_lin", C.c_int32), ("pad_", C.c_int32),
                ("g", C.c_void_p * MAX_LIN), ("v", C.c_void_p * MAX_LIN), ("b", C.c_void_p * MAX_LIN)]


MlpGrads = MlpParams


class RenderArgs(C.Structure):
    _fields_ = [
        ("B", C.c_int64), ("S", C.c_int32), ("n_lights", C.c_int32), ("flags", C.c_int32),
        ("cos_anneal_ratio", C.c_float),
        ("rays_o", C.c_void_p), ("rays_d", C.c_void_p), ("z_vals", C.c_void_p), ("lights_dir", C.c_void_p),
        ("background_rgb", C.c_void_p), ("variance", C.c_void_p),
        ("color_fine", C.c_void_p), ("weights", C.c_void_p), ("cdf_fine", C.c_void_p),
        ("gradients", C.c_void_p), ("inside_sphere", C.c_void_p), ("weight_sum", C.c_void_p),
        ("weight_max", C.c_void_p), ("s_val", C.c_void_p), ("gradient_error", C.c_void_p),
        ("sdf", C.c_void_p), ("sampled_albedo", C.c_void_p),
        ("gerr_partial", C.c_void_p), ("gerr_den_global", C.c_void_p),
    ]


class RenderMapsOut(C.Structure):
    _fields_ = [("color", C.c_void_p), ("normal", C.c_void_p), ("albedo", C.c_void_p), ("depth", C.c_void_p),
                ("weight_sum", C.c_void_p), ("weight_max", C.c_void_p)]


class GridDesc(C.Structure):
    _fields_ = [("bound_min", C.c_float * 3), ("bound_max", C.c_float * 3), ("resolution", C.c_int32),
                ("x_begin", C.c_int32), ("x_end", C.c_int32), ("out_scale", C.c_float)]


class SparseGridDesc(C.Structure):
    _fields_ = [("brick", C.c_int32), ("threshold", C.c_float), ("margin", C.c_float)]


class MeshVertexArgs(C.Structure):
    _fields_ = [("grid_vertices", C.c_void_p), ("points", C.c_void_p), ("V", C.c_int64),
                ("bound_min", C.c_float * 3), ("bound_max", C.c_float * 3), ("resolution", C.c_int32),
                ("level", C.c_float), ("refine", C.c_int32), ("max_step", C.c_float), ("flags", C.c_int32),
                ("points_out", C.c_void_p), ("sdf_out", C.c_void_p), ("gradient_out", C.c_void_p),
                ("normal_out", C.c_void_p), ("albedo_out", C.c_void_p), ("rgb_out", C.c_void_p)]


SPARSE_BRICKS = (4, 8, 16, 32)


def brick_geometry(res: int, brick: int) -> dict:
    res, brick = int(res), int(brick)
    if res < 2:
        raise ValueError(f"a grid of resolution {res} has no cells")
    if brick not in SPARSE_BRICKS:
        raise ValueError(f"brick must be one of {SPARSE_BRICKS}, not {brick}")
    nb = (res - 1 + brick - 1) // brick
    n1 = brick + 1
    return {"nb": nb, "lattice": [min(k * brick, res - 1) for k in range(nb + 1)], "samples": n1,
            "rows": (n1 ** 3 + 63) // 64 * 64, "bricks_total": nb ** 3}


SOURCE_U8, SOURCE_U16, SOURCE_F32 = 0, 1, 2


class SourceMaps(C.Structure):
    _fields_ = [("normals", C.c_void_p), ("albedo", C.c_void_p), ("mask", C.c_void_p), ("normals_type", C.c_int32),
                ("mask_type", C.c_int32), ("H", C.c_int32), ("W", C.c_int32), ("mask_channels", C.c_int32),
                ("n_lights", C.c_int32), ("local_lights", (C.c_float * 3) * MAX_RENDER_LIGHTS),
                ("warmup_lights_cam", (C.c_float * 3) * MAX_RENDER_LIGHTS)]


class RenderGrads(C.Structure):
    _fields_ = [("color_fine", C.c_void_p), ("weights", C.c_void_p), ("cdf_fine", C.c_void_p),
                ("gradients", C.c_void_p), ("weight_sum", C.c_void_p), ("weight_max", C.c_void_p),
                ("s_val", C.c_void_p), ("gradient_error", C.c_void_p)]


class RenderInputGrads(C.Structure):
    _fields_ = [("rays_o", C.c_void_p), ("rays_d", C.c_void_p), ("lights_dir", C.c_void_p),
                ("background_rgb", C.c_void_p), ("z_vals", C.c_void_p)]


_P = C.POINTER
_SIGNATURES = {
    "rnb_abi_version": (C.c_int, []),
    "rnb_last_error_string": (C.c_char_p, []),
    "rnb_build_id": (C.c_char_p, []),
    "rnb_packed_floats": (C.c_int, [_P(ModelDesc), _P(C.c_int64)]),
    "rnb_weightnorm_fwd": (C.c_int, [_P(ModelDesc), _P(MlpParams), _P(MlpParams), C.c_void_p, C.c_void_p]),
    "rnb_weightnorm_bwd": (C.c_int, [_P(ModelDesc), _P(MlpParams), _P(MlpParams), C.c_void_p, _P(MlpGrads),
                                     _P(MlpGrads), C.c_void_p]),
    "rnb_points_workspace_bytes": (C.c_int, [_P(ModelDesc), C.c_int64, _P(C.c_int64)]),
    "rnb_sdf_forward": (C.c_int, [_P(ModelDesc), C.c_void_p, C.c_void_p, C.c_int64, C.c_void_p, C.c_void_p,
                                  C.c_void_p, C.c_size_t, C.c_void_p]),
    "rnb_sdf_gradient": (C.c_int, [_P(ModelDesc), C.c_void_p, C.c_void_p, C.c_int64, C.c_void_p, C.c_void_p,
                                   C.c_void_p, C.c_size_t, C.c_void_p]),
    "rnb_color_forward": (C.c_int, [_P(ModelDesc), C.c_void_p, C.c_void_p, C.c_void_p, C.c_void_p, C.c_int64,
                                    C.c_void_p, C.c_void_p, C.c_size_t, C.c_void_p]),
    "rnb_points_grad_workspace_bytes": (C.c_int, [_P(ModelDesc), C.c_int64, C.c_int32, _P(C.c_int64)]),
    "rnb_sdf_forward_save": (C.c_int, [_P(ModelDesc), C.c_void_p, C.c_void_p, C.c_int64, C.c_int32, C.c_void_p,
                                       C.c_void_p, C.c_void_p, C.c_void_p, C.c_size_t, C.c_void_p]),
    "rnb_sdf_backward": (C.c_int, [_P(ModelDesc), C.c_void_p, C.c_int64, C.c_int32, C.c_void_p, C.c_void_p,
                                   C.c_void_p, C.c_void_p, C.c_void_p, C.c_void_p, C.c_size_t, C.c_void_p]),
    "rnb_color_forward_save": (C.c_int, [_P(ModelDesc), C.c_void_p, C.c_void_p, C.c_void_p, C.c_void_p, C.c_int64,
                                         C.c_void_p, C.c_void_p, C.c_size_t, C.c_void_p]),
    "rnb_color_backward": (C.c_int, [_P(ModelDesc), C.c_void_p, C.c_int64, C.c_void_p, C.c_void_p, C.c_void_p,
                                     C.c_void_p, C.c_void_p, C.c_void_p, C.c_size_t, C.c_void_p]),
    "rnb_sdf_grid_workspace_bytes": (C.c_int, [_P(ModelDesc), _P(GridDesc), _P(C.c_int64)]),
    "rnb_sdf_grid": (C.c_int, [_P(ModelDesc), C.c_void_p, _P(GridDesc), C.c_void_p, C.c_void_p, C.c_size_t,
                               C.c_void_p]),
    "rnb_sdf_grid_sparse_workspace_bytes": (C.c_int, [_P(ModelDesc), _P(GridDesc), _P(SparseGridDesc), _P(C.c_int64)]),
    "rnb_sdf_grid_sparse_seed": (C.c_int, [_P(ModelDesc), C.c_void_p, _P(GridDesc), _P(SparseGridDesc), C.c_void_p,
                                           C.c_size_t, C.c_void_p, C.c_void_p]),
    "rnb_sdf_grid_sparse_round": (C.c_int, [_P(ModelDesc), C.c_void_p, _P(GridDesc), _P(SparseGridDesc), C.c_void_p,
                                            C.c_void_p, C.c_size_t, C.c_int64, C.c_int64, C.c_void_p, C.c_void_p]),
    "rnb_sdf_grid_sparse_finish": (C.c_int, [_P(ModelDesc), _P(GridDesc), _P(SparseGridDesc), C.c_void_p, C.c_void_p,
                                             C.c_size_t, C.c_void_p, C.c_void_p]),
    "rnb_marching_cubes_workspace_bytes": (C.c_int, [C.c_int32, C.c_int32, C.c_int32, _P(C.c_int64)]),
    "rnb_marching_cubes_count": (C.c_int, [C.c_void_p, C.c_int32, C.c_int32, C.c_int32, C.c_float, C.c_void_p,
                                           C.c_size_t, C.c_void_p, C.c_void_p]),
    "rnb_marching_cubes_emit": (C.c_int, [C.c_void_p, C.c_int32, C.c_int32, C.c_int32, C.c_float, C.c_void_p,
                                          C.c_size_t, C.c_int64, C.c_int64, C.c_void_p, C.c_void_p, C.c_void_p]),
    "rnb_mesh_vertex_workspace_bytes": (C.c_int, [_P(ModelDesc), C.c_int64, C.c_int32, _P(C.c_int64)]),
    "rnb_mesh_vertex_attrs": (C.c_int, [_P(ModelDesc), C.c_void_p, _P(MeshVertexArgs), C.c_int64, C.c_void_p, C.c_size_t,
                                        C.c_void_p]),
    "rnb_up_sample_step": (C.c_int, [C.c_void_p, C.c_void_p, C.c_void_p, C.c_void_p, C.c_int64, C.c_int32,
                                     C.c_int32, C.c_float, C.c_void_p, C.c_void_p, C.c_void_p, C.c_void_p,
                                     C.c_void_p]),
    "rnb_gather_sdf": (C.c_int, [C.c_void_p, C.c_void_p, C.c_void_p, C.c_int64, C.c_int32, C.c_int32,
                                 C.c_void_p, C.c_void_p]),
    "rnb_sample_workspace_bytes": (C.c_int, [_P(ModelDesc), C.c_int64, _P(C.c_int64)]),
    "rnb_sample_rays": (C.c_int, [_P(ModelDesc), C.c_void_p, C.c_void_p, C.c_void_p, C.c_void_p, C.c_void_p,
                                  C.c_void_p, C.c_int64, C.c_void_p, C.c_void_p, C.c_size_t, C.c_void_p]),
    "rnb_render_workspace_bytes": (C.c_int, [_P(ModelDesc), C.c_int64, C.c_int32, C.c_int32, _P(C.c_int64)]),
    "rnb_render_fwd": (C.c_int, [_P(ModelDesc), C.c_void_p, _P(RenderArgs), C.c_void_p, C.c_size_t, C.c_void_p]),
    "rnb_render_maps": (C.c_int, [_P(ModelDesc), C.c_void_p, _P(RenderArgs), _P(RenderMapsOut), C.c_void_p, C.c_size_t,
                                  C.c_void_p]),
    "rnb_render_bwd": (C.c_int, [_P(ModelDesc), C.c_void_p, _P(RenderArgs), _P(RenderGrads), C.c_void_p,
                                 C.c_void_p, C.c_void_p, C.c_size_t, C.c_void_p]),
    "rnb_render_bwd_inputs": (C.c_int, [_P(ModelDesc), C.c_void_p, _P(RenderArgs), _P(RenderGrads),
                                        _P(RenderInputGrads), C.c_void_p, C.c_void_p, C.c_void_p, C.c_size_t,
                                        C.c_void_p]),
    "rnb_render_range": (C.c_int, [_P(ModelDesc), C.c_void_p, C.c_void_p, C.c_size_t, C.c_int64, C.c_int32, C.c_int32,
                                   C.c_void_p, C.c_void_p]),
    "rnb_algorithmic_flops": (C.c_int, [_P(ModelDesc), C.c_int64, C.c_int32, _P(C.c_double), _P(C.c_double)]),
    "rnb_algorithmic_bytes": (C.c_int, [_P(ModelDesc), C.c_int64, C.c_int32, _P(C.c_double)]),
    "rnb_gen_rays_at_view": (C.c_int, [C.c_void_p, C.c_void_p, C.c_void_p, C.c_void_p, C.c_void_p, C.c_int32,
                                       C.c_void_p, C.c_void_p, C.c_void_p, C.c_int64, C.c_int32, C.c_int32,
                                       C.c_int32, C.c_void_p, C.c_void_p, C.c_void_p, C.c_void_p, C.c_void_p,
                                       C.c_void_p, C.c_void_p]),
    "rnb_gen_rays_grid": (C.c_int, [C.c_void_p, C.c_void_p, C.c_void_p, C.c_void_p, C.c_int32, C.c_int32, C.c_int64,
                                    C.c_int64, C.c_void_p, C.c_void_p, C.c_void_p, C.c_int32, C.c_void_p, C.c_int32,
                                    C.c_int32, C.c_int32, C.c_int32, C.c_void_p, C.c_void_p, C.c_void_p, C.c_void_p,
                                    C.c_void_p, C.c_void_p, C.c_void_p]),
    "rnb_gen_rays_at_view_from_maps": (C.c_int, [C.c_void_p, C.c_void_p, _P(SourceMaps), C.c_void_p, C.c_void_p, C.c_int64,
                                                 C.c_void_p, C.c_void_p, C.c_void_p, C.c_void_p, C.c_void_p, C.c_void_p,
                                                 C.c_void_p]),
    "rnb_gen_rays_grid_from_maps": (C.c_int, [C.c_void_p, C.c_void_p, C.c_void_p, C.c_void_p, C.c_void_p, C.c_int32,
                                              C.c_int32, C.c_int64, C.c_int64, _P(SourceMaps), C.c_int32, C.c_void_p,
                                              C.c_void_p, C.c_void_p, C.c_void_p, C.c_void_p, C.c_void_p, C.c_void_p]),
    "rnb_gen_rays_camera_bwd": (C.c_int, [C.c_void_p, C.c_void_p, C.c_void_p, C.c_void_p, C.c_int64, C.c_void_p, C.c_int32,
                                          C.c_void_p, C.c_void_p, C.c_void_p, C.c_void_p, C.c_void_p, C.c_void_p, C.c_void_p,
                                          C.c_void_p]),
    "rnb_loss_rnb": (C.c_int, [C.c_void_p, C.c_void_p, C.c_void_p, C.c_void_p, C.c_void_p, C.c_int32, C.c_int64,
                               C.c_int32, C.c_float, C.c_float, C.c_void_p, C.c_void_p, C.c_void_p, C.c_void_p,
                               C.c_void_p, C.c_void_p]),
    "rnb_loss_rnb_shard": (C.c_int, [C.c_void_p, C.c_void_p, C.c_void_p, C.c_void_p, C.c_void_p, C.c_int32, C.c_int64,
                                     C.c_int32, C.c_float, C.c_float, C.c_void_p, C.c_float, C.c_void_p,
                                     C.c_void_p, C.c_void_p, C.c_void_p, C.c_void_p, C.c_void_p]),
    "rnb_adam_step": (C.c_int, [C.c_void_p, C.c_void_p, C.c_void_p, C.c_void_p, C.c_int64, C.c_double, C.c_double,
                                C.c_double, C.c_double, C.c_double, C.c_int64, C.c_void_p]),
    "rnb_profile_enable": (C.c_int, [C.c_int]),
    "rnb_profile_collect": (C.c_int, [_P(C.c_double), _P(C.c_int64), _P(C.c_double)]),
    "rnb_profile_report": (C.c_int64, [C.c_char_p, C.c_int64]),
}

EXPORTED_SYMBOLS = tuple(_SIGNATURES.keys())

_lib = None


class NativeError(RuntimeError):
    pass


def load():
    global _lib
    if _lib is not None:
        return _lib
    if not os.path.exists(LIB_PATH):
        raise NativeError(
            f"{LIB_PATH} is missing: build it with `python __graft_entry__.py` (hipcc, gfx950). "
            "There is no CPU fallback for the renderer.")
    lib = C.CDLL(LIB_PATH)
    for name, (restype, argtypes) in _SIGNATURES.items():
        try:
            fn = getattr(lib, name)
        except AttributeError as e:
            raise NativeError(f"{LIB_PATH} does not export {name}") from e
        fn.restype = restype
        fn.argtypes = argtypes
    v = lib.rnb_abi_version()
    if v != ABI_VERSION:
        raise NativeError(f"ABI version mismatch: library {v}, binding {ABI_VERSION}")
    _lib = lib
    return lib


def build_id() -> str:
    return load().rnb_build_id().decode()


def check(rc: int):
    if rc != 0:
        msg = load().rnb_last_error_string()
        raise NativeError(f"librnbneus_hip error {rc}: {msg.decode() if msg else '?'}")


def variant_bits(bf16=False, deterministic=False, generic=False, dw_lds=False, dw_staged=False, bwd_ti=0, bwd_nw=0,
                 fwd_ti=0, fwd_nw=0, x3=False, f32_mfma=False, reg_tile=False, lds_tile=False, x2h=None) -> int:
    nw = {0: 0, 4: 1, 8: 2}
    return ((VARIANT_BF16 if bf16 else 0) | (VARIANT_DETERMINISTIC if deterministic else 0)
            | (VARIANT_GENERIC if generic else 0) | (VARIANT_DW_LDS if dw_lds else 0)
            | (VARIANT_DW_STAGED if dw_staged else 0) | (VARIANT_X3 if x3 else 0) | (VARIANT_F32_MFMA if f32_mfma else 0)
            | (VARIANT_REG_TILE if reg_tile else 0) | (VARIANT_LDS_TILE if lds_tile else 0) | (0 if x2h is None else VARIANT_X2H if x2h else VARIANT_NO_X2H)
            | (int(bwd_ti) << VARIANT_BWD_TI_SHIFT) | (nw[int(bwd_nw)] << VARIANT_BWD_NW_SHIFT)
            | (int(fwd_ti) << VARIANT_FWD_TI_SHIFT) | (nw[int(fwd_nw)] << VARIANT_FWD_NW_SHIFT))


class on_device:

    def __init__(self, device):
        import torch
        if isinstance(device, torch.Tensor):
            device = device.device
        if device.type != "cuda":
            raise RuntimeError("librnbneus_hip.so works on GPU tensors only (there is no CPU path)")
        self._torch = torch
        self.device = device
        self._ctx = torch.cuda.device(device)

    def __enter__(self):
        self._ctx.__enter__()
        return C.c_void_p(self._torch.cuda.current_stream(self.device).cuda_stream)

    def __exit__(self, *exc):
        return self._ctx.__exit__(*exc)


def same_device(*tensors):
    dev = None
    for t in tensors:
        if t is None:
            continue
        if not t.is_cuda:
            raise RuntimeError("librnbneus_hip.so works on GPU tensors only (there is no CPU path)")
        if dev is None:
            dev = t.device
        elif t.device != dev:
            raise RuntimeError(f"tensors of one native call live on different devices ({dev} and {t.device})")
    return dev


def ptr(t):
    if t is None:
        return None
    assert t.is_contiguous(), "native call needs contiguous tensors"
    return C.c_void_p(t.data_ptr())
```

Baseline: 207,400 rays/s.

## Fuse fused RA and FB backward sweeps into a single chained kernel

Adds a fused_rafb kernel that runs the reverse-activation sweep and then the feature-backward sweep in the same block, sharing one LDS allocation. It is used when the route is x2h with TI=2, NW=4 tiles, and replaces two launches. The kernel bodies are moved into include files so both the standalone and chained kernels share the code. The SDF head backward now runs after both sweeps rather than between them, and a NO_CHAIN variant bit can disable the path. The intent is to cut launch overhead and improve cache locality between the sweeps, at the risk of higher register and LDS pressure in the combined kernel.

After: 205,700 rays/s. No clear change (-0.8%).

```diff
diff --git a/include/rnbneus.h b/include/rnbneus.h
--- a/include/rnbneus.h
+++ b/include/rnbneus.h
@@ -59,7 +59,8 @@
   RNB_VARIANT_REG_TILE = 1 << 16,
   RNB_VARIANT_LDS_TILE = 1 << 17,
   RNB_VARIANT_X2H = 1 << 18,
-  RNB_VARIANT_NO_X2H = 1 << 19
+  RNB_VARIANT_NO_X2H = 1 << 19,
+  RNB_VARIANT_NO_CHAIN = 1 << 20
 };
 
 typedef struct rnb_mlp_params {
diff --git a/rnb-neus-fork_amd/csrc/backward.hip b/rnb-neus-fork_amd/csrc/backward.hip
--- a/rnb-neus-fork_amd/csrc/backward.hip
+++ b/rnb-neus-fork_amd/csrc/backward.hip
@@ -192,7 +192,10 @@
     RNB_TRY(dw_backward(L, pb, dw_parts, 0, packed_grad, s));
   }
   int u_tiles = 0;
-  if (bf) {
+  const bool chain = !bf && parts.normal && r.sdf == SDF_FUSED && fused_rafb_runs(L, pb);
+  if (chain) {
+    RNB_TRY(fused_rafb(L, packed, pb, parts.feat, s, &u_tiles));
+  } else if (bf) {
     RNB_TRY(bf16_ra(L, packed, pb, s));
   } else if (!parts.normal) {
     for (int l = 0; l < L.nh; ++l) RNB_CHECK_HIP(hipMemsetAsync(pb.zR[l], 0, (size_t)pb.Mp * L.Hp * sizeof(float), s));
@@ -204,7 +207,7 @@
   int sdfh_slabs = 0;
   if (bf) RNB_TRY(bf16_sdf_head_bwd(L, pb, packed_grad, s));
   else RNB_TRY(launch_sdf_head_bwd(L, pb, parts.normal && r.sdf == SDF_LAYERS, u_tiles, packed_grad, &sdfh_slabs, s));
-  switch (r.sdf) {
+  if (!chain) switch (r.sdf) {
     case SDF_BF16: RNB_TRY(bf16_fb(L, packed, pb, parts.albedo, s)); break;
     case SDF_FUSED: RNB_TRY(fused_fb(L, packed, pb, parts.feat, s)); break;
     case SDF_LAYERS: RNB_TRY(layers_fb(L, packed, pb, parts.feat, s)); break;
diff --git a/rnb-neus-fork_amd/csrc/fused_bwd.hip b/rnb-neus-fork_amd/csrc/fused_bwd.hip
--- a/rnb-neus-fork_amd/csrc/fused_bwd.hip
+++ b/rnb-neus-fork_amd/csrc/fused_bwd.hip
@@ -185,125 +185,15 @@
   }
 }
 
+template <int TI>
+constexpr int ra_lds_floats() { return (TI == 1 ? 2 : 1) * 32 * TI * FP + 32 * TI * FEP; }
+
 template <int TI, int NW = 4, bool X3 = false>
 __global__ __launch_bounds__(64 * NW, (NW == 8 && TI == 2) ? 1 : 2) void fused_ra_kernel(FusedBwdArgs g) {
-  constexpr int BT = 32 * TI;
-  constexpr int NT = 64 * NW;
-  constexpr int TJ = 8 / NW;
-  [[maybe_unused]] constexpr bool BOTH_IN_LOOP = !(TI == 2 && TJ == 2);
-  constexpr int NBUF = TI == 1 ? 2 : 1;
-  __shared__ __attribute__((aligned(16))) float lds[NBUF * BT * FP + BT * FEP];
-  float* X = lds;
-  float* Y = lds + (NBUF - 1) * BT * FP;
-  float* E = lds + NBUF * BT * FP;
+  __shared__ __attribute__((aligned(16))) float lds[ra_lds_floats<TI>()];
   __shared__ float wmx[2][8];
-  const int tid = threadIdx.x, lane = tid & 63;
-  const int wave = wave_id();
-  const int64_t row0 = (int64_t)blockIdx.x * BT;
-  const int n0 = wave * 32 * TJ;
-
-  float gm = 0.f;
-  for (int idx = tid; idx < BT * g.net.Ep; idx += NT) {
-    const int r = idx / g.net.Ep, c = idx - r * g.net.Ep;
-    const float v = g.geb[(row0 + r) * g.net.Ep + c];
-    X[r * FP + c] = v;
-    if (c < FEP) E[r * FEP + c] = v;
-    gm = fmaxf(gm, fabsf(v));
-  }
-  if (g.amax != nullptr) {
-#pragma unroll
-    for (int o = 32; o > 0; o >>= 1) gm = fmaxf(gm, __shfl_xor(gm, o, 64));
-    if (lane == 0) wmx[1][wave] = gm;
-  }
-  __syncthreads();
-  if (g.amax != nullptr && tid == 0) {
-    float m = wmx[1][0];
-    for (int w = 1; w < NW; ++w) m = fmaxf(m, wmx[1][w]);
-    amax_tile_commit(g.amax + AMAX_U, m);
-  }
-
-  v16f acc[TI][TJ];
-  AuxTile<TI, TJ> aD, aG;
-  [[maybe_unused]] X3Mma<TI, TJ> mm;
-  if constexpr (X3 && !(TI == 2 && TJ == 2)) mm.request(g.w3 + 3 * g.net.w_off[0], g.net.Kp[0], n0, lane);
-  for (int l = 0; l < g.net.nh; ++l) {
-    layer_mma<TI, TJ, X3>(X, g, g.net.w_off[l], g.net.Kp[l], n0, lane, acc, mm, l + 1 < g.net.nh ? g.net.w_off[l + 1] : -1,
-                     [&]() {
-                       if constexpr (!(X3 && !BOTH_IN_LOOP)) prefetch_tile<TI, TJ>(g.D[l], row0, n0, lane, aD);
-                       if constexpr (BOTH_IN_LOOP) prefetch_tile<TI, TJ>(g.gz[l], row0, n0, lane, aG);
-                     });
-    const int lane_e = opaque_lane(lane);
-    const int h = lane_e >> 5;
-    if constexpr (X3 && !BOTH_IN_LOOP) prefetch_tile<TI, TJ>(g.D[l], row0, n0, lane_e, aD);
-    if constexpr (!BOTH_IN_LOOP) prefetch_tile<TI, TJ>(g.gz[l], row0, n0, lane_e, aG);
-    if constexpr (NBUF == 1) lds_barrier();
-    const int n_real = g.net.n_real[l];
-    const bool pe_tail = (l + 1 == g.net.skip);
-    const BufRsrc rzR = tile_rsrc(g.zR[l] + (size_t)row0 * FH, BT * FH * 4);
-    if (l + 1 == g.net.nh && g.ucol != nullptr) {
-      float cs[TJ];
-#pragma unroll
-      for (int tj = 0; tj < TJ; ++tj) cs[tj] = 0.f;
-      for_each_acc<TI, TJ>(n0, lane_e, [&](int tj, int ti, int r, int col, int rowc, int row) {
-        const float v = acc[ti][tj][r];
-        const float un = col < n_real ? v * aD.v[ti][tj][r] : 0.f;
-        const float zr = col < n_real ? ((v - un) * aG.v[ti][tj][r]) * 100.f : 0.f;
-        bstore(rzR, (unsigned)(4 * h * FH + col) * 4u, rowc * FH * 4, zr);
-        cs[tj] += (row0 + row < g.M) ? un : 0.f;
-      });
-#pragma unroll
-      for (int tj = 0; tj < TJ; ++tj) {
-        const float tot = cs[tj] + __shfl_xor(cs[tj], 32, 64);
-        if (lane_e < 32) g.ucol[(size_t)blockIdx.x * FH + n0 + tj * 32 + lane_e] = tot;
-      }
-      break;
-    }
-    const BufRsrc ru = tile_rsrc(g.u[l + 1] + (size_t)row0 * FH, BT * FH * 4);
-    float um[2] = {0.f, 0.f};
-    for_each_acc_split<TI, TJ>(
-        n0, lane_e, n_real,
-        [&](int tj, int ti, int r, int col, int rowc, int row) {
-          const unsigned voff = (unsigned)(4 * h * FH + col) * 4u;
-          const unsigned soff = rowc * FH * 4;
-          const float v = acc[ti][tj][r];
-          const float un = v * aD.v[ti][tj][r];
-          const float zr = ((v - un) * aG.v[ti][tj][r]) * 100.f;
-          Y[row * FP + col] = un;
-          bstore(rzR, voff, soff, zr);
-          bstore(ru, voff, soff, un);
-          um[r & 1] = fmaxf(um[r & 1], fabsf(un));
-        },
-        [&](int tj, int ti, int r, int col, int rowc, int row) {
-          const unsigned voff = (unsigned)(4 * h * FH + col) * 4u;
-          const unsigned soff = rowc * FH * 4;
-          const float v = acc[ti][tj][r];
-          float zr, un;
-          if (col < n_real) {
-            un = v * aD.v[ti][tj][r];
-            zr = ((v - un) * aG.v[ti][tj][r]) * 100.f;
-          } else {
-            zr = 0.f;
-            un = (pe_tail && col < n_real + g.net.pe) ? E[row * FEP + (col - n_real)] : 0.f;
-          }
-          Y[row * FP + col] = un;
-          bstore(rzR, voff, soff, zr);
-          bstore(ru, voff, soff, un);
-          um[r & 1] = fmaxf(um[r & 1], fabsf(un));
-        });
-    if (g.amax != nullptr) {
-      float m = fmaxf(um[0], um[1]);
-#pragma unroll
-      for (int o = 32; o > 0; o >>= 1) m = fmaxf(m, __shfl_xor(m, o, 64));
-      if (lane_e == 0) wmx[l & 1][wave] = m;
-    }
-    lds_barrier();
-    if (g.amax != nullptr && tid == 0) {
-      float m = wmx[l & 1][0];
-      for (int w = 1; w < NW; ++w) m = fmaxf(m, wmx[l & 1][w]);
-      amax_tile_commit(g.amax + AMAX_U + l + 1, m);
-    }
-    if constexpr (NBUF == 2) { float* t = X; X = Y; Y = t; }
-  }
+  const int tid = threadIdx.x;
+#include "fused_ra_body.inc"
 }
 
 template <int TI, int NW = 4, bool X3 = false>
@@ -393,109 +283,27 @@
 
 template <int NW>
 __global__ __launch_bounds__(64 * NW, NW == 8 ? 1 : 2) void fused_fb_h2_kernel(FusedBwdArgs g) {
-  constexpr int TI = 2, BT = 64, NT = 64 * NW, TJ = 8 / NW;
-  __shared__ __attribute__((aligned(16))) float lds[BT * FP];
+  __shared__ __attribute__((aligned(16))) float lds[64 * FP];
   __shared__ float wm[2][8];
-  float* X = lds;
-  const int tid = threadIdx.x, lane = tid & 63;
-  const int wave = wave_id();
-  const int64_t row0 = (int64_t)blockIdx.x * BT;
-  const int n0 = wave * 32 * TJ;
-  const long long left = g.M - row0;
-  const int rows_ok = left >= BT ? BT : (int)(left < 0 ? 0 : left);
-
-  v16f acc[TI][TJ];
-  AuxTile<TI, TJ> aD, aZ;
-  X3Mma<TI, TJ, 2> mm;
-  constexpr bool LATE = TJ == 2;
-  if constexpr (!LATE) {
-    if (g.fbar != nullptr) mm.request(g.w3 + 2 * g.net.wfT_off, FH, n0, lane);
-    else if (g.net.nh > 1) mm.request(g.w3 + 2 * g.net.wT_off[g.net.nh - 1], FH, n0, lane);
-    prefetch_tile<TI, TJ>(g.D[g.net.nh - 1], row0, n0, lane, aD);
-    prefetch_tile<TI, TJ>(g.zR[g.net.nh - 1], row0, n0, lane, aZ);
-  }
-  for (int ti_ = 0; ti_ < TI; ++ti_) for (int tj_ = 0; tj_ < TJ; ++tj_) for (int r_ = 0; r_ < 16; ++r_) acc[ti_][tj_][r_] = 0.f;
-  float unscale = 1.f;
-  const float iwsv = h2_iws_load(g.h2tab, lane);
-  if (g.fbar != nullptr) {
-    const float* fb = g.fbar + (size_t)row0 * g.ld_fbar;
-    float m = 0.f;
-    for (int idx = tid; idx < BT * FH / 4; idx += NT) {
-      const int r = idx >> 6, c4 = idx & 63;
-      const vf4 v = *reinterpret_cast<const vf4*>(fb + (size_t)r * g.ld_fbar + c4 * 4);
-      *reinterpret_cast<vf4*>(X + r * FP + c4 * 4) = v;
-      if (r < rows_ok) m = fmaxf(fmaxf(m, fmaxf(fabsf(v.x), fabsf(v.y))), fmaxf(fabsf(v.z), fabsf(v.w)));
-    }
-    m = wave_max(m);
-    if (lane == 0) wm[1][wave] = m;
-    __syncthreads();
-    float s, inv;
-    tile_scale<NW>(wm[1], s, inv);
-    for (int idx = tid; idx < BT * FH / 4; idx += NT) {
-      const int r = idx >> 6, c4 = idx & 63;
-      vf4* q = reinterpret_cast<vf4*>(X + r * FP + c4 * 4);
-      *q = *q * s;
-    }
-    __syncthreads();
-    if constexpr (LATE) mm.request(g.w3 + 2 * g.net.wfT_off, FH, n0, lane);
-    mm.run(X, g.w3 + 2 * g.net.wfT_off, FH, n0, lane, acc, (!LATE && g.net.nh > 1) ? g.w3 + 2 * g.net.wT_off[g.net.nh - 1] : nullptr, FH, n0);
-    unscale = inv * h2_iws_at(iwsv, g.net.nh);
-  }
-  if constexpr (LATE) {
-    prefetch_tile<TI, TJ>(g.D[g.net.nh - 1], row0, n0, lane, aD);
-    prefetch_tile<TI, TJ>(g.zR[g.net.nh - 1], row0, n0, lane, aZ);
-  }
-  for (int l = g.net.nh - 1; l >= 0; --l) {
-    const int lane_e = opaque_lane(lane);
-    const int h = lane_e >> 5;
-    const int n_real = g.net.n_real[l];
-    const bool head = (l == g.net.nh - 1);
-    const int par = l & 1;
-    const BufRsrc rzb = tile_rsrc(g.zb[l] + (size_t)row0 * FH, BT * FH * 4);
-    if (head) {
-      for_each_acc<TI, TJ>(n0, lane_e, [&](int tj, int ti, int r, int col, int rowc, int row) {
-        acc[ti][tj][r] = fmaf(g.sbar[row0 + row] * g.net.inv_scale, g.packed[g.net.wsdf_off + col], acc[ti][tj][r] * unscale);
-      });
-      unscale = 1.f;
-    }
-    for_each_acc_split<TI, TJ>(
-        n0, lane_e, n_real,
-        [&](int tj, int ti, int r, int col, int rowc, int row) {
-          const float zb = fmaf(acc[ti][tj][r] * unscale, aD.v[ti][tj][r], aZ.v[ti][tj][r]);
-          bstore(rzb, (unsigned)(4 * h * FH + col) * 4u, rowc * FH * 4, zb);
-          acc[ti][tj][r] = zb;
-        },
-        [&](int tj, int ti, int r, int col, int rowc, int row) {
-          const float zb = col < n_real ? fmaf(acc[ti][tj][r] * unscale, aD.v[ti][tj][r], aZ.v[ti][tj][r]) : 0.f;
-          bstore(rzb, (unsigned)(4 * h * FH + col) * 4u, rowc * FH * 4, zb);
-          acc[ti][tj][r] = zb;
-        });
-    {
-      const float mr = wave_max(acc_absmax<TI, TJ>(acc, lane_e, rows_ok));
-      if (lane_e == 0) wm[par][wave] = mr;
-    }
-    lds_barrier();
-    float s, inv;
-    const float tmax = tile_scale<NW>(wm[par], s, inv);
-    if (tid == 0 && g.amax != nullptr) amax_tile_commit(g.amax + AMAX_ZB + l, tmax);
-    if (l == 0) break;
-    for_each_acc<TI, TJ>(n0, lane_e, [&](int tj, int ti, int r, int col, int rowc, int row) {
-      X[row * FP + col] = acc[ti][tj][r] * s;
-    });
-    lds_barrier();
-    if constexpr (LATE) {
-      mm.request(g.w3 + 2 * g.net.wT_off[l], FH, n0, lane);
-      mm.run(X, g.w3 + 2 * g.net.wT_off[l], FH, n0, lane, acc, nullptr, 0, 0);
-      prefetch_tile<TI, TJ>(g.D[l - 1], row0, n0, opaque_lane(lane), aD);
-      prefetch_tile<TI, TJ>(g.zR[l - 1], row0, n0, opaque_lane(lane), aZ);
-    } else {
-      mm.run(X, g.w3 + 2 * g.net.wT_off[l], FH, n0, lane, acc, l > 1 ? g.w3 + 2 * g.net.wT_off[l - 1] : nullptr, FH, n0, [&]() {
-        prefetch_tile<TI, TJ>(g.D[l - 1], row0, n0, lane, aD);
-        prefetch_tile<TI, TJ>(g.zR[l - 1], row0, n0, lane, aZ);
-      });
-    }
-    unscale = inv * h2_iws_at(iwsv, l);
-  }
+#include "fused_fb_h2_body.inc"
+}
+
+template <int NW>
+__global__ __launch_bounds__(64 * NW, 2) void fused_rafb_kernel(FusedBwdArgs ga, FusedBwdArgs gf) {
+  static_assert(ra_lds_floats<2>() >= 64 * FP, "one allocation, sized to the larger body");
+  __shared__ __attribute__((aligned(16))) float lds[ra_lds_floats<2>()];
+  __shared__ float wm[2][8];
+  {
+    constexpr int TI = 2;
+    constexpr bool X3 = true;
+    const FusedBwdArgs& g = ga;
+    float (&wmx)[2][8] = wm;
+    const int tid = opaque_lane(threadIdx.x);
+#include "fused_ra_body.inc"
+  }
+  __syncthreads();
+  const FusedBwdArgs& g = gf;
+#include "fused_fb_h2_body.inc"
 }
 
 static void fill_args(const Layout& L, const float* packed, PointBufs& pb, FusedBwdArgs& g) {
@@ -587,4 +395,31 @@
   return RNB_OK;
 }
 
-}
+bool fused_rafb_runs(const Layout& L, const PointBufs& pb) {
+  if ((L.variant & RNB_VARIANT_NO_CHAIN) || !is_x2h(L)) return false;
+  bool ok = false;
+  pick_tile(L, pb, [&](auto ti_c, auto nw_c, dim3, dim3) { ok = decltype(ti_c)::value == 2 && decltype(nw_c)::value == 4; });
+  return ok;
+}
+
+int fused_rafb(const Layout& L, const float* packed, PointBufs& pb, bool with_color, hipStream_t s, int* u_tiles) {
+  if (!fused_rafb_runs(L, pb)) RNB_FAIL(RNB_E_INVALID, "fused_rafb: this model's route launches RA and FB separately");
+  FusedBwdArgs ga, gf;
+  fill_args(L, packed, pb, ga);
+  ga.ucol = pb.u[L.nh];
+  gf = ga;
+  gf.ucol = nullptr;
+  gf.fbar = with_color ? pb.cinb : nullptr;
+  gf.ld_fbar = L.Cinp;
+  gf.w3 = x2h_mirror(L, packed);
+  const dim3 grid((unsigned)(pb.Mp / 64)), block(256);
+  *u_tiles = (int)grid.x;
+  ProfScope prof(sdf_sweep_flops(L, pb.M, 0, false, false) + sdf_sweep_flops(L, pb.M, 1, false, with_color), s, "RA+FB_sweep");
+  hipLaunchKernelGGL((fused_rafb_kernel<4>), grid, block, 0, s, ga, gf);
+  prof_ran("RA_sweep");
+  prof_ran("FB_sweep");
+  RNB_CHECK_LAUNCH();
+  return RNB_OK;
+}
+
+}
diff --git a/rnb-neus-fork_amd/csrc/fused_fb_h2_body.inc b/rnb-neus-fork_amd/csrc/fused_fb_h2_body.inc
--- /dev/null
+++ b/rnb-neus-fork_amd/csrc/fused_fb_h2_body.inc
@@ -0,0 +1,101 @@
+  constexpr int TI = 2, BT = 64, NT = 64 * NW, TJ = 8 / NW;
+  float* X = lds;
+  const int tid = threadIdx.x, lane = tid & 63;
+  const int wave = wave_id();
+  const int64_t row0 = (int64_t)blockIdx.x * BT;
+  const int n0 = wave * 32 * TJ;
+  const long long left = g.M - row0;
+  const int rows_ok = left >= BT ? BT : (int)(left < 0 ? 0 : left);
+
+  v16f acc[TI][TJ];
+  AuxTile<TI, TJ> aD, aZ;
+  X3Mma<TI, TJ, 2> mm;
+  constexpr bool LATE = TJ == 2;
+  if constexpr (!LATE) {
+    if (g.fbar != nullptr) mm.request(g.w3 + 2 * g.net.wfT_off, FH, n0, lane);
+    else if (g.net.nh > 1) mm.request(g.w3 + 2 * g.net.wT_off[g.net.nh - 1], FH, n0, lane);
+    prefetch_tile<TI, TJ>(g.D[g.net.nh - 1], row0, n0, lane, aD);
+    prefetch_tile<TI, TJ>(g.zR[g.net.nh - 1], row0, n0, lane, aZ);
+  }
+  for (int ti_ = 0; ti_ < TI; ++ti_) for (int tj_ = 0; tj_ < TJ; ++tj_) for (int r_ = 0; r_ < 16; ++r_) acc[ti_][tj_][r_] = 0.f;
+  float unscale = 1.f;
+  const float iwsv = h2_iws_load(g.h2tab, lane);
+  if (g.fbar != nullptr) {
+    const float* fb = g.fbar + (size_t)row0 * g.ld_fbar;
+    float m = 0.f;
+    for (int idx = tid; idx < BT * FH / 4; idx += NT) {
+      const int r = idx >> 6, c4 = idx & 63;
+      const vf4 v = *reinterpret_cast<const vf4*>(fb + (size_t)r * g.ld_fbar + c4 * 4);
+      *reinterpret_cast<vf4*>(X + r * FP + c4 * 4) = v;
+      if (r < rows_ok) m = fmaxf(fmaxf(m, fmaxf(fabsf(v.x), fabsf(v.y))), fmaxf(fabsf(v.z), fabsf(v.w)));
+    }
+    m = wave_max(m);
+    if (lane == 0) wm[1][wave] = m;
+    __syncthreads();
+    float s, inv;
+    tile_scale<NW>(wm[1], s, inv);
+    for (int idx = tid; idx < BT * FH / 4; idx += NT) {
+      const int r = idx >> 6, c4 = idx & 63;
+      vf4* q = reinterpret_cast<vf4*>(X + r * FP + c4 * 4);
+      *q = *q * s;
+    }
+    __syncthreads();
+    if constexpr (LATE) mm.request(g.w3 + 2 * g.net.wfT_off, FH, n0, lane);
+    mm.run(X, g.w3 + 2 * g.net.wfT_off, FH, n0, lane, acc, (!LATE && g.net.nh > 1) ? g.w3 + 2 * g.net.wT_off[g.net.nh - 1] : nullptr, FH, n0);
+    unscale = inv * h2_iws_at(iwsv, g.net.nh);
+  }
+  if constexpr (LATE) {
+    prefetch_tile<TI, TJ>(g.D[g.net.nh - 1], row0, n0, lane, aD);
+    prefetch_tile<TI, TJ>(g.zR[g.net.nh - 1], row0, n0, lane, aZ);
+  }
+  for (int l = g.net.nh - 1; l >= 0; --l) {
+    const int lane_e = opaque_lane(lane);
+    const int h = lane_e >> 5;
+    const int n_real = g.net.n_real[l];
+    const bool head = (l == g.net.nh - 1);
+    const int par = l & 1;
+    const BufRsrc rzb = tile_rsrc(g.zb[l] + (size_t)row0 * FH, BT * FH * 4);
+    if (head) {
+      for_each_acc<TI, TJ>(n0, lane_e, [&](int tj, int ti, int r, int col, int rowc, int row) {
+        acc[ti][tj][r] = fmaf(g.sbar[row0 + row] * g.net.inv_scale, g.packed[g.net.wsdf_off + col], acc[ti][tj][r] * unscale);
+      });
+      unscale = 1.f;
+    }
+    for_each_acc_split<TI, TJ>(
+        n0, lane_e, n_real,
+        [&](int tj, int ti, int r, int col, int rowc, int row) {
+          const float zb = fmaf(acc[ti][tj][r] * unscale, aD.v[ti][tj][r], aZ.v[ti][tj][r]);
+          bstore(rzb, (unsigned)(4 * h * FH + col) * 4u, rowc * FH * 4, zb);
+          acc[ti][tj][r] = zb;
+        },
+        [&](int tj, int ti, int r, int col, int rowc, int row) {
+          const float zb = col < n_real ? fmaf(acc[ti][tj][r] * unscale, aD.v[ti][tj][r], aZ.v[ti][tj][r]) : 0.f;
+          bstore(rzb, (unsigned)(4 * h * FH + col) * 4u, rowc * FH * 4, zb);
+          acc[ti][tj][r] = zb;
+        });
+    {
+      const float mr = wave_max(acc_absmax<TI, TJ>(acc, lane_e, rows_ok));
+      if (lane_e == 0) wm[par][wave] = mr;
+    }
+    lds_barrier();
+    float s, inv;
+    const float tmax = tile_scale<NW>(wm[par], s, inv);
+    if (tid == 0 && g.amax != nullptr) amax_tile_commit(g.amax + AMAX_ZB + l, tmax);
+    if (l == 0) break;
+    for_each_acc<TI, TJ>(n0, lane_e, [&](int tj, int ti, int r, int col, int rowc, int row) {
+      X[row * FP + col] = acc[ti][tj][r] * s;
+    });
+    lds_barrier();
+    if constexpr (LATE) {
+      mm.request(g.w3 + 2 * g.net.wT_off[l], FH, n0, lane);
+      mm.run(X, g.w3 + 2 * g.net.wT_off[l], FH, n0, lane, acc, nullptr, 0, 0);
+      prefetch_tile<TI, TJ>(g.D[l - 1], row0, n0, opaque_lane(lane), aD);
+      prefetch_tile<TI, TJ>(g.zR[l - 1], row0, n0, opaque_lane(lane), aZ);
+    } else {
+      mm.run(X, g.w3 + 2 * g.net.wT_off[l], FH, n0, lane, acc, l > 1 ? g.w3 + 2 * g.net.wT_off[l - 1] : nullptr, FH, n0, [&]() {
+        prefetch_tile<TI, TJ>(g.D[l - 1], row0, n0, lane, aD);
+        prefetch_tile<TI, TJ>(g.zR[l - 1], row0, n0, lane, aZ);
+      });
+    }
+    unscale = inv * h2_iws_at(iwsv, l);
+  }
diff --git a/rnb-neus-fork_amd/csrc/fused_ra_body.inc b/rnb-neus-fork_amd/csrc/fused_ra_body.inc
--- /dev/null
+++ b/rnb-neus-fork_amd/csrc/fused_ra_body.inc
@@ -0,0 +1,115 @@
+  constexpr int BT = 32 * TI;
+  constexpr int NT = 64 * NW;
+  constexpr int TJ = 8 / NW;
+  [[maybe_unused]] constexpr bool BOTH_IN_LOOP = !(TI == 2 && TJ == 2);
+  constexpr int NBUF = TI == 1 ? 2 : 1;
+  float* X = lds;
+  float* Y = lds + (NBUF - 1) * BT * FP;
+  float* E = lds + NBUF * BT * FP;
+  const int lane = tid & 63;
+  const int wave = wave_id();
+  const int64_t row0 = (int64_t)blockIdx.x * BT;
+  const int n0 = wave * 32 * TJ;
+
+  float gm = 0.f;
+  for (int idx = tid; idx < BT * g.net.Ep; idx += NT) {
+    const int r = idx / g.net.Ep, c = idx - r * g.net.Ep;
+    const float v = g.geb[(row0 + r) * g.net.Ep + c];
+    X[r * FP + c] = v;
+    if (c < FEP) E[r * FEP + c] = v;
+    gm = fmaxf(gm, fabsf(v));
+  }
+  if (g.amax != nullptr) {
+#pragma unroll
+    for (int o = 32; o > 0; o >>= 1) gm = fmaxf(gm, __shfl_xor(gm, o, 64));
+    if (lane == 0) wmx[1][wave] = gm;
+  }
+  __syncthreads();
+  if (g.amax != nullptr && tid == 0) {
+    float m = wmx[1][0];
+    for (int w = 1; w < NW; ++w) m = fmaxf(m, wmx[1][w]);
+    amax_tile_commit(g.amax + AMAX_U, m);
+  }
+
+  v16f acc[TI][TJ];
+  AuxTile<TI, TJ> aD, aG;
+  [[maybe_unused]] X3Mma<TI, TJ> mm;
+  if constexpr (X3 && !(TI == 2 && TJ == 2)) mm.request(g.w3 + 3 * g.net.w_off[0], g.net.Kp[0], n0, lane);
+  for (int l = 0; l < g.net.nh; ++l) {
+    layer_mma<TI, TJ, X3>(X, g, g.net.w_off[l], g.net.Kp[l], n0, lane, acc, mm, l + 1 < g.net.nh ? g.net.w_off[l + 1] : -1,
+                     [&]() {
+                       if constexpr (!(X3 && !BOTH_IN_LOOP)) prefetch_tile<TI, TJ>(g.D[l], row0, n0, lane, aD);
+                       if constexpr (BOTH_IN_LOOP) prefetch_tile<TI, TJ>(g.gz[l], row0, n0, lane, aG);
+                     });
+    const int lane_e = opaque_lane(lane);
+    const int h = lane_e >> 5;
+    if constexpr (X3 && !BOTH_IN_LOOP) prefetch_tile<TI, TJ>(g.D[l], row0, n0, lane_e, aD);
+    if constexpr (!BOTH_IN_LOOP) prefetch_tile<TI, TJ>(g.gz[l], row0, n0, lane_e, aG);
+    if constexpr (NBUF == 1) lds_barrier();
+    const int n_real = g.net.n_real[l];
+    const bool pe_tail = (l + 1 == g.net.skip);
+    const BufRsrc rzR = tile_rsrc(g.zR[l] + (size_t)row0 * FH, BT * FH * 4);
+    if (l + 1 == g.net.nh && g.ucol != nullptr) {
+      float cs[TJ];
+#pragma unroll
+      for (int tj = 0; tj < TJ; ++tj) cs[tj] = 0.f;
+      for_each_acc<TI, TJ>(n0, lane_e, [&](int tj, int ti, int r, int col, int rowc, int row) {
+        const float v = acc[ti][tj][r];
+        const float un = col < n_real ? v * aD.v[ti][tj][r] : 0.f;
+        const float zr = col < n_real ? ((v - un) * aG.v[ti][tj][r]) * 100.f : 0.f;
+        bstore(rzR, (unsigned)(4 * h * FH + col) * 4u, rowc * FH * 4, zr);
+        cs[tj] += (row0 + row < g.M) ? un : 0.f;
+      });
+#pragma unroll
+      for (int tj = 0; tj < TJ; ++tj) {
+        const float tot = cs[tj] + __shfl_xor(cs[tj], 32, 64);
+        if (lane_e < 32) g.ucol[(size_t)blockIdx.x * FH + n0 + tj * 32 + lane_e] = tot;
+      }
+      break;
+    }
+    const BufRsrc ru = tile_rsrc(g.u[l + 1] + (size_t)row0 * FH, BT * FH * 4);
+    float um[2] = {0.f, 0.f};
+    for_each_acc_split<TI, TJ>(
+        n0, lane_e, n_real,
+        [&](int tj, int ti, int r, int col, int rowc, int row) {
+          const unsigned voff = (unsigned)(4 * h * FH + col) * 4u;
+          const unsigned soff = rowc * FH * 4;
+          const float v = acc[ti][tj][r];
+          const float un = v * aD.v[ti][tj][r];
+          const float zr = ((v - un) * aG.v[ti][tj][r]) * 100.f;
+          Y[row * FP + col] = un;
+          bstore(rzR, voff, soff, zr);
+          bstore(ru, voff, soff, un);
+          um[r & 1] = fmaxf(um[r & 1], fabsf(un));
+        },
+        [&](int tj, int ti, int r, int col, int rowc, int row) {
+          const unsigned voff = (unsigned)(4 * h * FH + col) * 4u;
+          const unsigned soff = rowc * FH * 4;
+          const float v = acc[ti][tj][r];
+          float zr, un;
+          if (col < n_real) {
+            un = v * aD.v[ti][tj][r];
+            zr = ((v - un) * aG.v[ti][tj][r]) * 100.f;
+          } else {
+            zr = 0.f;
+            un = (pe_tail && col < n_real + g.net.pe) ? E[row * FEP + (col - n_real)] : 0.f;
+          }
+          Y[row * FP + col] = un;
+          bstore(rzR, voff, soff, zr);
+          bstore(ru, voff, soff, un);
+          um[r & 1] = fmaxf(um[r & 1], fabsf(un));
+        });
+    if (g.amax != nullptr) {
+      float m = fmaxf(um[0], um[1]);
+#pragma unroll
+      for (int o = 32; o > 0; o >>= 1) m = fmaxf(m, __shfl_xor(m, o, 64));
+      if (lane_e == 0) wmx[l & 1][wave] = m;
+    }
+    lds_barrier();
+    if (g.amax != nullptr && tid == 0) {
+      float m = wmx[l & 1][0];
+      for (int w = 1; w < NW; ++w) m = fmaxf(m, wmx[l & 1][w]);
+      amax_tile_commit(g.amax + AMAX_U + l + 1, m);
+    }
+    if constexpr (NBUF == 2) { float* t = X; X = Y; Y = t; }
+  }
diff --git a/rnb-neus-fork_amd/csrc/layout.hip b/rnb-neus-fork_amd/csrc/layout.hip
--- a/rnb-neus-fork_amd/csrc/layout.hip
+++ b/rnb-neus-fork_amd/csrc/layout.hip
@@ -41,7 +41,7 @@
   if (d->sdf_multires < 0 || d->sdf_multires > 16) RNB_FAIL(RNB_E_INVALID, "bad sdf_multires");
   if (!(d->sdf_scale > 0.f)) RNB_FAIL(RNB_E_INVALID, "sdf_scale must be positive");
   L->variant = d->variant;
-  if (d->variant & ~0xFFF7F) RNB_FAIL(RNB_E_INVALID, "unknown bits in rnb_model_desc.variant (0x%x)", d->variant);
+  if (d->variant & ~0x1FFF7F) RNB_FAIL(RNB_E_INVALID, "unknown bits in rnb_model_desc.variant (0x%x)", d->variant);
   L->nh = d->sdf_n_layers;
   L->multires = d->sdf_multires;
   L->pe = 3 * (1 + 2 * d->sdf_multires);
diff --git a/rnb-neus-fork_amd/csrc/prof.hip b/rnb-neus-fork_amd/csrc/prof.hip
--- a/rnb-neus-fork_amd/csrc/prof.hip
+++ b/rnb-neus-fork_amd/csrc/prof.hip
@@ -13,6 +13,7 @@
   size_t used = 0;
   std::vector<double> flops;
   std::vector<const char*> tag;
+  std::vector<const char*> ran;
 };
 static ProfState g_prof;
 
@@ -37,11 +38,16 @@
   p.used += 2;
 }
 
+void prof_ran(const char* tag) {
+  if (g_prof.on) g_prof.ran.push_back(tag);
+}
+
 int profile_enable(int on) {
   g_prof.on = on != 0;
   g_prof.used = 0;
   g_prof.flops.clear();
   g_prof.tag.clear();
+  g_prof.ran.clear();
   return RNB_OK;
 }
 
@@ -66,12 +72,18 @@
     g_classes[c].flops += p.flops[i];
     g_classes[c].n += 1;
   }
+  for (const char* tg : p.ran) {
+    size_t c = 0;
+    while (c < g_classes.size() && strcmp(g_classes[c].tag, tg) != 0) ++c;
+    if (c == g_classes.size()) g_classes.push_back(ProfClass{tg, 0.0, 0.0, 0});
+  }
   if (ms) *ms = t;
   if (launches) *launches = (int64_t)n;
   if (flops) *flops = f;
   p.used = 0;
   p.flops.clear();
   p.tag.clear();
+  p.ran.clear();
   return RNB_OK;
 }
 
diff --git a/rnb-neus-fork_amd/csrc/rnb_internal.h b/rnb-neus-fork_amd/csrc/rnb_internal.h
--- a/rnb-neus-fork_amd/csrc/rnb_internal.h
+++ b/rnb-neus-fork_amd/csrc/rnb_internal.h
@@ -362,6 +362,8 @@
 int fused_reverse(const Layout& L, const float* packed, PointBufs& pb, hipStream_t s, bool store_ge = false);
 int fused_ra(const Layout& L, const float* packed, PointBufs& pb, hipStream_t s, int* u_tiles = nullptr);
 int fused_fb(const Layout& L, const float* packed, PointBufs& pb, bool with_color, hipStream_t s);
+bool fused_rafb_runs(const Layout& L, const PointBufs& pb);
+int fused_rafb(const Layout& L, const float* packed, PointBufs& pb, bool with_color, hipStream_t s, int* u_tiles);
 
 bool fused_supported(const Layout& L);
 int fused_forward(const Layout& L, const float* packed, const float* pts, int64_t M, PointBufs& pb, bool save,
@@ -528,6 +530,7 @@
 bool prof_enabled();
 void prof_begin(double flops, hipStream_t s, const char* tag);
 void prof_end(hipStream_t s);
+void prof_ran(const char* tag);
 int profile_enable(int on);
 int profile_collect(double* ms, int64_t* launches, double* flops);
 int64_t profile_report(char* out, int64_t cap);
diff --git a/rnb-neus-fork_amd/native.py b/rnb-neus-fork_amd/native.py
--- a/rnb-neus-fork_amd/native.py
+++ b/rnb-neus-fork_amd/native.py
@@ -36,6 +36,7 @@
 VARIANT_LDS_TILE = 1 << 17
 VARIANT_X2H = 1 << 18
 VARIANT_NO_X2H = 1 << 19
+VARIANT_NO_CHAIN = 1 << 20
 
 c_float_p = C.c_void_p
 
@@ -270,12 +271,13 @@
 
 
 def variant_bits(bf16=False, deterministic=False, generic=False, dw_lds=False, dw_staged=False, bwd_ti=0, bwd_nw=0,
-                 fwd_ti=0, fwd_nw=0, x3=False, f32_mfma=False, reg_tile=False, lds_tile=False, x2h=None) -> int:
+                 fwd_ti=0, fwd_nw=0, x3=False, f32_mfma=False, reg_tile=False, lds_tile=False, x2h=None, chain=True) -> int:
     nw = {0: 0, 4: 1, 8: 2}
     return ((VARIANT_BF16 if bf16 else 0) | (VARIANT_DETERMINISTIC if deterministic else 0)
             | (VARIANT_GENERIC if generic else 0) | (VARIANT_DW_LDS if dw_lds else 0)
             | (VARIANT_DW_STAGED if dw_staged else 0) | (VARIANT_X3 if x3 else 0) | (VARIANT_F32_MFMA if f32_mfma else 0)
             | (VARIANT_REG_TILE if reg_tile else 0) | (VARIANT_LDS_TILE if lds_tile else 0) | (0 if x2h is None else VARIANT_X2H if x2h else VARIANT_NO_X2H)
+            | (0 if chain else VARIANT_NO_CHAIN)
             | (int(bwd_ti) << VARIANT_BWD_TI_SHIFT) | (nw[int(bwd_nw)] << VARIANT_BWD_NW_SHIFT)
             | (int(fwd_ti) << VARIANT_FWD_TI_SHIFT) | (nw[int(fwd_nw)] << VARIANT_FWD_NW_SHIFT))
 
```
